# ilovepose/fast-human-pose-estimation.pytorch

Measured on AMD Instinct MI355X. Metric: images/sec FPD train step (4-stack HG student, 8-stack teacher) 256x256, higher is better.
Workload: dtype bf16; 1 GPU; configs[1]: hourglass student S=4 F=128 + teacher S=8 F=256, 256x256, batch 32/GPU, fused FPD step incl. Adam, teacher forward one batch ahead on a 2nd stream; global_batch=32, parallelism=dp1, backend=mfma, launch=one native plan call per phase, kernels launched eagerly on 3 streams, ranks=1, finite=True

## Files before the change

### fast-human-pose-estimation.pytorch_amd/csrc/api.hip

```cpp
#include <cstdarg>
#include <cstdio>
#include <cstdlib>
#include <cstring>
#include <string>
#include <vector>

#include "conv_dispatch.h"

int g_fpd_backend = FPD_BACKEND_MFMA;
static thread_local char g_err[512] = "";

static FILE* g_launch_log_file = nullptr;
static bool launch_log_open() {
    const char* path = getenv("FPD_LAUNCH_LOG");
    if (path == nullptr || path[0] == 0) return false;
    g_launch_log_file = fopen(path, "w");
    if (g_launch_log_file == nullptr) fprintf(stderr, "[fpd_amd] FPD_LAUNCH_LOG: cannot open %s\n", path);
    return g_launch_log_file != nullptr;
}
bool g_fpd_launch_log = launch_log_open();
static thread_local char g_op_tag[256] = "-";
void fpd_log_launch(const char* kernel, const dim3& grid, const dim3& block) {
    if (g_launch_log_file == nullptr) return;
    fprintf(g_launch_log_file, "%s\t%u\t%u\t%s\n", kernel, grid.x * grid.y * grid.z, block.x * block.y * block.z, g_op_tag);
    fflush(g_launch_log_file);
}

int fpd_fail(int code, const char* fmt, ...) {
    va_list ap;
    va_start(ap, fmt);
    vsnprintf(g_err, sizeof(g_err), fmt, ap);
    va_end(ap);
    return code;
}

static int check_launch() {
    hipError_t e = hipGetLastError();
    if (e != hipSuccess) return fpd_fail(-100 - (int)e, "kernel launch failed: %s", hipGetErrorString(e));
    return 0;
}

static int validate_conv_dims(int N, int H, int W, int C, int K, int R, int S, int stride, int pad, int P, int Q) {
    FPD_REQUIRE(N > 0 && H > 0 && W > 0 && C > 0 && K > 0 && R > 0 && S > 0 && stride > 0 && pad >= 0,
                "conv: non-positive dimension");
    FPD_REQUIRE(P == (H + 2 * pad - R) / stride + 1 && Q == (W + 2 * pad - S) / stride + 1,
                "conv: output %dx%d inconsistent with input %dx%d k=%dx%d stride=%d pad=%d", P, Q, H, W, R, S, stride, pad);
    FPD_REQUIRE((int64_t)N * H * W * C < (1ll << 31) && (int64_t)N * P * Q * K < (1ll << 31), "conv: tensor too large for 32-bit indexing");
    return 0;
}

extern "C" {

const char* fpd_last_error(void) { return g_err; }
int fpd_abi_version(void) { return FPD_ABI_VERSION; }
int64_t fpd_stats_words(int32_t channels) { return FPD_STATS_WORDS(channels); }
int fpd_set_backend(int32_t backend) {
    const int prev = g_fpd_backend;
    if (backend == FPD_BACKEND_MFMA || backend == FPD_BACKEND_NAIVE || backend == FPD_BACKEND_MFMA_GENERIC) g_fpd_backend = backend;
    return prev;
}

static int g_wgrad_tile_only = 0;

int fpd_set_option(const char* name, int32_t value) {
    FPD_REQUIRE(name, "set_option: null name");
    if (!strcmp(name, "conv_pp")) return fpd_conv_pp_option(0, value);
    if (!strcmp(name, "conv_pp_blocks")) return fpd_conv_pp_option(1, value);
    if (!strcmp(name, "conv_c1")) return fpd_conv_c1_option(0, value);
    if (!strcmp(name, "conv_c1_blocks")) return fpd_conv_c1_option(1, value);
    if (!strcmp(name, "conv_c1_launches")) return fpd_conv_c1_option(2, value);
    if (!strcmp(name, "conv_skip")) return fpd_conv_c1_option(3, value);
    if (!strcmp(name, "stem_act")) return fpd_stem_s2d_option(0, value);
    if (!strcmp(name, "ew_merge")) return fpd_ew_merge_option(value < 0 ? 0 : value);
    if (!strcmp(name, "ew_merge_blocks")) return fpd_ew_merge_blocks_option(value);
    if (!strcmp(name, "ew_blocks")) return fpd_ew_blocks_option(value);
    if (!strcmp(name, "conv_c3")) return fpd_conv_c3_option(0, value);
    if (!strcmp(name, "conv_c3_blocks")) return fpd_conv_c3_option(1, value);
    if (!strcmp(name, "conv_c3_launches")) return fpd_conv_c3_option(2, value);
    if (!strcmp(name, "bneck_blocks")) return fpd_bneck_blocks_option(value);
    if (!strcmp(name, "bneck_upadd")) return fpd_bneck_upadd_option(value);
    if (!strcmp(name, "head_blocks")) return fpd_head_blocks_option(value);
    if (!strcmp(name, "wgrad_tile_only")) { g_wgrad_tile_only = value; return 0; }
    return fpd_fail(-2, "set_option: unknown option '%s'", name);
}

int fpd_abi_sizeof(const char* n) {
#define SZ(T) if (!strcmp(n, #T)) return (int)sizeof(T)
    SZ(fpd_bn_t); SZ(fpd_conv_t); SZ(fpd_wgrad_t); SZ(fpd_stem_t); SZ(fpd_ew_t); SZ(fpd_loss_t); SZ(fpd_adam_t);
    SZ(fpd_wprep_entry_t); SZ(fpd_bnupd_entry_t); SZ(fpd_memset_t); SZ(fpd_table_t); SZ(fpd_wreduce_entry_t); SZ(fpd_bneck_t); SZ(fpd_conv_pair_t); SZ(fpd_bneck_pair_t); SZ(fpd_ew_pair_t); SZ(fpd_pck_t); SZ(fpd_head_t); SZ(fpd_affsum_t); SZ(fpd_layout_t);
    SZ(fpd_conv_f8_t); SZ(fpd_wquant_entry_t); SZ(fpd_flipmerge_t); SZ(fpd_finalpreds_t); SZ(fpd_targets_t); SZ(fpd_warp_src_t); SZ(fpd_warp_t);
    SZ(fpd_loss_ohkm_t); SZ(fpd_sgd_t); SZ(fpd_ew_merge_t); SZ(fpd_loss_kl_t);
    SZ(fpd_aug_img_t); SZ(fpd_aug_db_t); SZ(fpd_aug_crop_t); SZ(fpd_augment_t); SZ(fpd_warp_aug_t); SZ(fpd_targets_w_t); SZ(fpd_targets_unbiased_t);
    SZ(fpd_oks_nms_t); SZ(fpd_coco_match_t); SZ(fpd_coco_accum_t); SZ(fpd_val_post_t); SZ(fpd_dark_t);
    SZ(fpd_vis_minmax_t); SZ(fpd_vis_max_preds_t); SZ(fpd_vis_joints_grid_t); SZ(fpd_vis_heatmap_grid_t);
#undef SZ
    return -1;
}

static int validate_conv(const fpd_conv_t* a) {
    FPD_REQUIRE(a && a->x && a->w && a->y, "conv: null pointer");
    int rc = validate_conv_dims(a->N, a->H, a->W, a->C, a->K, a->R, a->S, a->stride, a->pad, a->P, a->Q);
    if (rc) return rc;
    FPD_REQUIRE(a->dtype == FPD_F32 || a->dtype == FPD_BF16, "conv: bad dtype %d", a->dtype);
    FPD_REQUIRE(a->bn.mode == FPD_BN_NONE || (a->bn.gamma && a->bn.beta), "conv: BN prologue without gamma/beta");
    FPD_REQUIRE(a->bn.mode != FPD_BN_TRAIN || a->bn.stats, "conv: train-mode BN without statistics");
    FPD_REQUIRE(a->bn.mode != FPD_BN_EVAL || (a->bn.running_mean && a->bn.running_var), "conv: eval-mode BN without running stats");
    FPD_REQUIRE(a->epi == FPD_EPI_PLAIN || (a->epi_x && a->epi_stats && a->epi_bn.mode == FPD_BN_TRAIN && a->epi_bn.stats),
                "conv: BNRELU_BWD epilogue needs epi_x, epi_stats and a train-mode epi_bn");
    FPD_REQUIRE(a->x2 == nullptr || (a->w2 != nullptr && a->C2 > 0), "conv: a second source (x2) needs w2 and C2");
    FPD_REQUIRE(a->x2 == nullptr || a->residual == nullptr, "conv: a second source (x2) and a residual exclude each other");
    return 0;
}

constexpr unsigned ON_MFMA = 1u << FPD_BACKEND_MFMA, ON_GENERIC = ON_MFMA | 1u << FPD_BACKEND_MFMA_GENERIC, ON_ANY = ON_GENERIC | 1u << FPD_BACKEND_NAIVE;
struct ConvBackend {
    const char* name;
    unsigned backends;
    int (*route)(const fpd_conv_t& a, const fpd_conv_t* b, ConvAsk ask, ConvRoute& r);
    int (*launch)(const fpd_conv_t& a, const fpd_conv_t* b, hipStream_t st);
};
static const ConvBackend g_conv_backends[] = {
    {"conv_c1", ON_MFMA, fpd_conv_c1_route, fpd_conv_c1_launch},
    {"conv_c3", ON_MFMA, fpd_conv_c3_route, fpd_conv_c3_launch},
    {"conv_pp", ON_MFMA, fpd_conv_pp_route, fpd_conv_pp_launch},
    {"conv_tile", ON_MFMA, fpd_conv_tile_route, fpd_conv_tile_launch},
    {"conv_mfma", ON_GENERIC, nullptr, [](const fpd_conv_t& a, const fpd_conv_t*, hipStream_t st) { return fpd_conv_mfma_launch(a, st); }},
    {"conv_smallc", ON_GENERIC, nullptr, [](const fpd_conv_t& a, const fpd_conv_t*, hipStream_t st) { return fpd_conv_smallc_launch(a, st); }},
    {"conv_naive", ON_ANY, nullptr, [](const fpd_conv_t& a, const fpd_conv_t*, hipStream_t st) { return fpd_conv_naive_launch(a, st); }},
};
static bool eligible(unsigned backends) { return (backends >> g_fpd_backend & 1u) != 0; }

static const ConvBackend* route_conv(const fpd_conv_t& a, const fpd_conv_t* b, ConvAsk ask, ConvRoute& r) {
    r = ConvRoute{false, 0, 0, false};
    for (const ConvBackend& e : g_conv_backends) {
        if (!eligible(e.backends)) continue;
        if (e.route == nullptr ? b == nullptr : e.route(a, b, ask, r) == 0) return &e;
    }
    return nullptr;
}

static int launch_conv(const fpd_conv_t& a, const fpd_conv_t* b, hipStream_t st) {
    ConvRoute r;
    const ConvBackend* e = route_conv(a, b, fpd_conv_ask(a, b), r);
    if (e == nullptr) {
        const int rc = launch_conv(a, nullptr, st);
        return rc ? rc : launch_conv(*b, nullptr, st);
    }
    FPD_REQUIRE(!(a.wg_partial != nullptr && r.slabs_a == 0) && !(b != nullptr && b->wg_partial != nullptr && r.slabs_b == 0),
                "conv: the launch asks for a fused weight gradient (wg_partial), which its route (%s) does not offer; %s() reports 0 for it",
                e->name, b ? "fpd_conv_pair_fused_wgrad_partials" : "fpd_conv_fused_wgrad_partials");
    FPD_REQUIRE(r.folds || (a.fold_x == nullptr && (b == nullptr || b->fold_x == nullptr)),
                "conv: the launch asks for a folded BN-backward apply (fold_x), which its route (%s) does not offer; %s() reports 0 for it",
                e->name, b ? "fpd_conv_pair_fold_supported" : "fpd_conv_fold_supported");
    FPD_REQUIRE(r.skips || (a.x2 == nullptr && (b == nullptr || b->x2 == nullptr)),
                "conv: the launch carries a second 1x1 source (x2), which its route (%s) does not offer; fpd_conv_skip_supported() reports 0 for it", e->name);
    int rc = e->launch(a, b, st);
    for (++e; rc == 1 && e != std::end(g_conv_backends); ++e)
        if (e->route == nullptr && eligible(e->backends)) rc = e->launch(a, b, st);
    return rc;
}

int fpd_conv_forward(const fpd_conv_t* a, fpd_stream_t stream) {
    int rc = validate_conv(a);
    if (rc) return rc;
    rc = launch_conv(*a, nullptr, (hipStream_t)stream);
    return rc ? rc : check_launch();
}

int fpd_conv_fold_supported(const fpd_conv_t* a) {
    ConvRoute r;
    if (!a || validate_conv(a) != 0) return 0;
    route_conv(*a, nullptr, ConvAsk{true, a->wg_partial != nullptr, a->x2 != nullptr}, r);
    return r.folds ? 1 : 0;
}
int fpd_conv_pair_fold_supported(const fpd_conv_pair_t* p) {
    ConvRoute r;
    if (!p || validate_conv(&p->a) != 0 || validate_conv(&p->b) != 0) return 0;
    if (route_conv(p->a, &p->b, ConvAsk{true, fpd_conv_ask(p->a, &p->b).wg, fpd_conv_ask(p->a, &p->b).skip}, r) != nullptr) return r.folds ? 1 : 0;
    return (fpd_conv_fold_supported(&p->a) && fpd_conv_fold_supported(&p->b)) ? 1 : 0;
}

int fpd_conv_skip_supported(const fpd_conv_t* a) {
    ConvRoute r;
    if (!a || validate_conv(a) != 0) return 0;
    route_conv(*a, nullptr, ConvAsk{a->fold_x != nullptr, a->wg_partial != nullptr, true}, r);
    return r.skips ? 1 : 0;
}

int fpd_conv_fused_wgrad_partials(const fpd_conv_t* a) {
    ConvRoute r;
    if (!a || validate_conv(a) != 0) return 0;
    route_conv(*a, nullptr, ConvAsk{a->fold_x != nullptr, true, a->x2 != nullptr}, r);
    return r.slabs_a;
}
int fpd_conv_pair_fused_wgrad_partials(const fpd_conv_pair_t* p, int32_t* n_a, int32_t* n_b) {
    FPD_REQUIRE(p && n_a && n_b, "conv_pair_fused_wgrad_partials: null pointer");
    *n_a = *n_b = 0;
    if (validate_conv(&p->a) != 0 || validate_conv(&p->b) != 0) return 0;
    ConvRoute r;
    route_conv(p->a, &p->b, ConvAsk{fpd_conv_ask(p->a, &p->b).fold, true, fpd_conv_ask(p->a, &p->b).skip}, r);
    *n_a = r.slabs_a; *n_b = r.slabs_b;
    return 0;
}

int fpd_conv_f8_in_domain(const fpd_conv_t* c) { return (c && fpd_conv_f8_domain(*c)) ? 1 : 0; }

int fpd_conv_forward_f8(const fpd_conv_f8_t* a, fpd_stream_t stream) {
    FPD_REQUIRE(a, "conv_f8: null pointer");
    int rc = validate_conv(&a->c);
    if (rc) return rc;
    FPD_REQUIRE(a->w8 && a->w8_scale, "conv_f8: null fp8 weights / scales");
    FPD_REQUIRE(((uintptr_t)a->w8 & 15) == 0, "conv_f8: w8 must be 16-byte aligned");
    rc = 1;
    if (g_fpd_backend == FPD_BACKEND_MFMA) rc = fpd_conv_tile_f8_launch(a->c, a->w8, a->w8_scale, (hipStream_t)stream);
    if (rc == 1) rc = launch_conv(a->c, nullptr, (hipStream_t)stream);
    return rc ? rc : check_launch();
}

int fpd_weight_quant_f8(const fpd_wquant_entry_t* t, int32_t n, fpd_stream_t stream) {
    FPD_REQUIRE(n == 0 || t != nullptr, "weight_quant_f8: null table");
    int rc = fpd_weight_quant_f8_launch(t, n, (hipStream_t)stream);
    return rc ? rc : check_launch();
}

int fpd_conv_forward_pair(const fpd_conv_pair_t* p, fpd_stream_t stream) {
    FPD_REQUIRE(p, "conv_pair: null pointer");
// ... 513 lines not shown
    return rc ? rc : check_launch();
}

int fpd_weight_prep(const fpd_wprep_entry_t* t, int32_t n, int64_t max_elems, int32_t dtype, fpd_stream_t stream) {
    int rc = fpd_weight_prep_launch(t, n, max_elems, dtype, (hipStream_t)stream);
    return rc ? rc : check_launch();
}
int fpd_bn_update_running(const fpd_bnupd_entry_t* t, int32_t n, fpd_stream_t stream) {
    int rc = fpd_bn_update_running_launch(t, n, (hipStream_t)stream);
    return rc ? rc : check_launch();
}
int fpd_cast(const void* src, void* dst, int64_t n, int32_t sd, int32_t dd, fpd_stream_t stream) {
    int rc = fpd_cast_launch(src, dst, n, sd, dd, (hipStream_t)stream);
    return rc ? rc : check_launch();
}
int fpd_nchw_to_nhwc(const float* src, void* dst, int32_t N, int32_t C, int32_t H, int32_t W, int32_t dtype, fpd_stream_t stream) {
    int rc = fpd_nchw_to_nhwc_launch(src, dst, N, C, H, W, dtype, (hipStream_t)stream);
    return rc ? rc : check_launch();
}
int fpd_nhwc_to_nchw(const void* src, float* dst, int32_t N, int32_t C, int32_t H, int32_t W, int32_t dtype, fpd_stream_t stream) {
    int rc = fpd_nhwc_to_nchw_launch(src, dst, N, C, H, W, dtype, (hipStream_t)stream);
    return rc ? rc : check_launch();
}

struct fpd_op {
    int32_t type;
    union {
        fpd_affsum_t affsum; fpd_layout_t layout; fpd_conv_f8_t conv8; fpd_conv_t conv; fpd_conv_pair_t pair; fpd_bneck_t bneck; fpd_bneck_pair_t bpair; fpd_ew_pair_t epair; fpd_pck_t pck; fpd_head_t head; fpd_wgrad_t wgrad; fpd_stem_t stem; fpd_ew_t ew; fpd_loss_t loss; fpd_loss_ohkm_t lossk; fpd_loss_kl_t losskl; fpd_adam_t adam; fpd_sgd_t sgd; fpd_ew_merge_t ewm;
        fpd_memset_t mset; fpd_table_t table;
    } u;
};
struct fpd_sched {
    int32_t lane = 0;
    bool record = false;
    hipEvent_t done = nullptr;
    std::vector<int32_t> waits;
};
struct fpd_plan {
    std::vector<fpd_op> ops;
    std::vector<fpd_sched> sched;
    std::vector<hipGraphExec_t> graphs;
    std::vector<hipGraph_t> graph_defs;
    hipStream_t lanes[FPD_MAX_LANES] = {};
    hipEvent_t lane_done[FPD_MAX_LANES] = {};
    hipEvent_t fork = nullptr;
};

fpd_plan* fpd_plan_create(void) { return new fpd_plan(); }
void fpd_plan_destroy(fpd_plan* p) {
    if (!p) return;
    for (auto g : p->graphs) (void)hipGraphExecDestroy(g);
    for (auto g : p->graph_defs) (void)hipGraphDestroy(g);
    for (auto& s : p->sched) if (s.done) (void)hipEventDestroy(s.done);
    for (int l = 0; l < FPD_MAX_LANES; ++l) {
        if (p->lanes[l]) (void)hipStreamDestroy(p->lanes[l]);
        if (p->lane_done[l]) (void)hipEventDestroy(p->lane_done[l]);
    }
    if (p->fork) (void)hipEventDestroy(p->fork);
    delete p;
}
int fpd_plan_size(const fpd_plan* p) { return p ? (int)p->ops.size() : -1; }

int fpd_plan_add(fpd_plan* p, int32_t op, const void* args, int64_t bytes) {
    FPD_REQUIRE(p && args, "plan_add: null");
    fpd_op o;
    memset(&o, 0, sizeof(o));
    o.type = op;
    size_t want = 0;
    switch (op) {
        case FPD_OP_CONV: want = sizeof(fpd_conv_t); break;
        case FPD_OP_CONV_F8: want = sizeof(fpd_conv_f8_t); break;
        case FPD_OP_WGRAD: want = sizeof(fpd_wgrad_t); break;
        case FPD_OP_CONV_PAIR: want = sizeof(fpd_conv_pair_t); break;
        case FPD_OP_BNECK_PAIR: want = sizeof(fpd_bneck_pair_t); break;
        case FPD_OP_EW_PAIR: want = sizeof(fpd_ew_pair_t); break;
        case FPD_OP_PCK: want = sizeof(fpd_pck_t); break;
        case FPD_OP_HEAD: case FPD_OP_HEAD_FOLD: want = sizeof(fpd_head_t); break;
        case FPD_OP_BNECK: case FPD_OP_BNECK_FOLD: want = sizeof(fpd_bneck_t); break;
        case FPD_OP_STEM_FWD: case FPD_OP_STEM_WGRAD: want = sizeof(fpd_stem_t); break;
        case FPD_OP_EW: want = sizeof(fpd_ew_t); break;
        case FPD_OP_EW_MERGE: want = sizeof(fpd_ew_merge_t); break;
        case FPD_OP_LOSS: want = sizeof(fpd_loss_t); break;
        case FPD_OP_LOSS_OHKM: want = sizeof(fpd_loss_ohkm_t); break;
        case FPD_OP_LOSS_KL: want = sizeof(fpd_loss_kl_t); break;
        case FPD_OP_ADAM: want = sizeof(fpd_adam_t); break;
        case FPD_OP_SGD: want = sizeof(fpd_sgd_t); break;
        case FPD_OP_MEMSET: case FPD_OP_NOP: want = sizeof(fpd_memset_t); break;
        case FPD_OP_AFFSUM: want = sizeof(fpd_affsum_t); break;
        case FPD_OP_NCHW2NHWC: want = sizeof(fpd_layout_t); break;
        case FPD_OP_WPREP: case FPD_OP_BNUPD: case FPD_OP_WREDUCE: case FPD_OP_WQUANT: want = sizeof(fpd_table_t); break;
        default: return fpd_fail(-2, "plan_add: unknown op %d", op);
    }
    FPD_REQUIRE((size_t)bytes == want, "plan_add: op %d expects %zu bytes of args, got %lld", op, want, (long long)bytes);
    memcpy(&o.u, args, want);
    p->ops.push_back(o);
    p->sched.emplace_back();
    return (int)p->ops.size() - 1;
}

int fpd_plan_set_schedule(fpd_plan* p, int32_t op, int32_t lane, const int32_t* wait_ops, int32_t n_waits) {
    FPD_REQUIRE(p && op >= 0 && op < (int)p->ops.size(), "plan_set_schedule: bad op index %d", op);
    FPD_REQUIRE(lane >= 0 && lane < FPD_MAX_LANES, "plan_set_schedule: lane %d outside [0,%d)", lane, FPD_MAX_LANES);
    FPD_REQUIRE(n_waits >= 0 && (n_waits == 0 || wait_ops != nullptr), "plan_set_schedule: bad wait list");
    for (int i = 0; i < n_waits; ++i)
        FPD_REQUIRE(wait_ops[i] >= 0 && wait_ops[i] < op, "plan_set_schedule: op %d may only wait for earlier ops (got %d)", op, wait_ops[i]);
    fpd_sched& s = p->sched[op];
    s.lane = lane;
    s.waits.assign(wait_ops, wait_ops + n_waits);
    for (int i = 0; i < n_waits; ++i) p->sched[wait_ops[i]].record = true;
    return 0;
}

int fpd_plan_mark_event(fpd_plan* p, int32_t op) {
    FPD_REQUIRE(p && op >= 0 && op < (int)p->ops.size(), "plan_mark_event: bad op index %d", op);
    p->sched[op].record = true;
    return 0;
}

int fpd_plan_wait_op(fpd_plan* p, int32_t op, fpd_stream_t stream) {
    FPD_REQUIRE(p && op >= 0 && op < (int)p->ops.size(), "plan_wait_op: bad op index %d", op);
    FPD_REQUIRE(p->sched[op].record && p->sched[op].done, "plan_wait_op: op %d has no recorded event (mark it, then run its range)", op);
    FPD_CHECK_HIP(hipStreamWaitEvent((hipStream_t)stream, p->sched[op].done, 0));
    return 0;
}

static void conv_tag(char* p, size_t n, const char* what, const fpd_conv_t& c) {
    snprintf(p, n, "%s N=%d H=%d W=%d C=%d K=%d R=%d s=%d %s%s%s%s%s", what, c.N, c.H, c.W, c.C, c.K, c.R, c.stride,
             c.epi == FPD_EPI_BNRELU_BWD ? "dgrad" : "fwd", c.bn.mode == FPD_BN_EVAL ? " evalbn" : "", c.wg_partial ? " +wgrad" : "", c.fold_x ? " +fold" : "",
             c.x2 ? " +skip" : "");
}
static void set_op_tag(int idx, const fpd_op& o) {
    char t[200] = "";
    static const char* ew_names[] = {"bnrelu_fwd", "bnrelu_bwd_r", "bn_bwd_apply", "maxpool_fwd", "maxpool_bwd", "upadd_fwd", "sumpool", "add", "relu_mask", "dilate2"};
    auto ewn = [&](int op) { return (op >= 0 && op < 10) ? ew_names[op] : "ew"; };
    switch (o.type) {
        case FPD_OP_CONV: conv_tag(t, sizeof(t), "conv", o.u.conv); break;
        case FPD_OP_CONV_F8: conv_tag(t, sizeof(t), "conv_f8", o.u.conv8.c); break;
        case FPD_OP_CONV_PAIR: {
            char a[90], b[90];
            conv_tag(a, sizeof(a), "conv2", o.u.pair.a);
            snprintf(b, sizeof(b), " | H=%d W=%d", o.u.pair.b.H, o.u.pair.b.W);
            snprintf(t, sizeof(t), "%s%s", a, b);
            break;
        }
        case FPD_OP_WGRAD: snprintf(t, sizeof(t), "wgrad N=%d H=%d W=%d C=%d K=%d R=%d s=%d", o.u.wgrad.N, o.u.wgrad.H, o.u.wgrad.W, o.u.wgrad.C, o.u.wgrad.K, o.u.wgrad.R, o.u.wgrad.stride); break;
        case FPD_OP_BNECK: snprintf(t, sizeof(t), "bneck N=%d H=%d W=%d C=%d P=%d%s", o.u.bneck.N, o.u.bneck.H, o.u.bneck.W, o.u.bneck.C, o.u.bneck.P, o.u.bneck.x2 ? "+upadd" : ""); break;
        case FPD_OP_BNECK_PAIR: snprintf(t, sizeof(t), "bneck2 N=%d H=%d W=%d C=%d P=%d | H=%d W=%d", o.u.bpair.a.N, o.u.bpair.a.H, o.u.bpair.a.W, o.u.bpair.a.C, o.u.bpair.a.P, o.u.bpair.b.H, o.u.bpair.b.W); break;
        case FPD_OP_HEAD: snprintf(t, sizeof(t), "head N=%d H=%d W=%d C=%d J=%d", o.u.head.N, o.u.head.H, o.u.head.W, o.u.head.C, o.u.head.J); break;
        case FPD_OP_EW: snprintf(t, sizeof(t), "ew %s N=%d H=%d W=%d C=%d", ewn(o.u.ew.op), o.u.ew.N, o.u.ew.H, o.u.ew.W, o.u.ew.C); break;
        case FPD_OP_EW_PAIR: snprintf(t, sizeof(t), "ew2 %s N=%d H=%d W=%d C=%d | H=%d W=%d", ewn(o.u.epair.a.op), o.u.epair.a.N, o.u.epair.a.H, o.u.epair.a.W, o.u.epair.a.C, o.u.epair.b.H, o.u.epair.b.W); break;
        case FPD_OP_EW_MERGE: {
            const fpd_ew_merge_t& m = o.u.ewm;
            const bool pb = m.kind == FPD_EWM_MAXPOOL_BWD;
            snprintf(t, sizeof(t), "ewm %s N=%d H=%d W=%d C=%d", pb ? (m.has_full ? "apply2+maxpool_bwd" : "apply+maxpool_bwd") : "apply+sumpool", m.pool.N, m.pool.H, m.pool.W, m.pool.C);
            break;
        }
        case FPD_OP_STEM_FWD: case FPD_OP_STEM_WGRAD: snprintf(t, sizeof(t), "%s N=%d H=%d W=%d K=%d%s", o.type == FPD_OP_STEM_FWD ? "stem_fwd" : "stem_wgrad", o.u.stem.N, o.u.stem.H, o.u.stem.W, o.u.stem.K,
                                                              (o.type == FPD_OP_STEM_FWD && o.u.stem.act.mode != FPD_BN_NONE) ? " +act" : ""); break;
        case FPD_OP_AFFSUM: snprintf(t, sizeof(t), "affsum N=%d H=%d W=%d C=%d terms=%d", o.u.affsum.N, o.u.affsum.H, o.u.affsum.W, o.u.affsum.C, o.u.affsum.nterms); break;
        case FPD_OP_LOSS: snprintf(t, sizeof(t), "loss B=%d J=%d H=%d W=%d S=%d", o.u.loss.B, o.u.loss.J, o.u.loss.H, o.u.loss.W, o.u.loss.S); break;
        case FPD_OP_LOSS_OHKM: snprintf(t, sizeof(t), "loss_ohkm B=%d J=%d H=%d W=%d S=%d k=%d,%d", o.u.lossk.base.B, o.u.lossk.base.J, o.u.lossk.base.H, o.u.lossk.base.W, o.u.lossk.base.S, o.u.lossk.topk_pose, o.u.lossk.topk_kd); break;
        case FPD_OP_LOSS_KL: snprintf(t, sizeof(t), "loss_kl B=%d J=%d H=%d W=%d S=%d kl=%d,%d T=%g,%g", o.u.losskl.base.B, o.u.losskl.base.J, o.u.losskl.base.H, o.u.losskl.base.W, o.u.losskl.base.S, o.u.losskl.kl_pose, o.u.losskl.kl_kd, (double)o.u.losskl.temp_pose, (double)o.u.losskl.temp_kd); break;
        case FPD_OP_ADAM: snprintf(t, sizeof(t), "adam n=%lld", (long long)o.u.adam.n); break;
        case FPD_OP_SGD: snprintf(t, sizeof(t), "sgd n=%lld momentum=%g wd=%g%s", (long long)o.u.sgd.n, (double)o.u.sgd.momentum, (double)o.u.sgd.weight_decay, o.u.sgd.nesterov ? " nesterov" : ""); break;
        case FPD_OP_WREDUCE: snprintf(t, sizeof(t), "wreduce entries=%d", o.u.table.n); break;
        case FPD_OP_WPREP: snprintf(t, sizeof(t), "wprep entries=%d", o.u.table.n); break;
        case FPD_OP_BNUPD: snprintf(t, sizeof(t), "bnupd entries=%d", o.u.table.n); break;
        default: snprintf(t, sizeof(t), "op%d", o.type); break;
    }
    snprintf(g_op_tag, sizeof(g_op_tag), "%d\t%s", idx, t);
}

static int run_op(const fpd_op& o, fpd_stream_t s) {
    switch (o.type) {
        case FPD_OP_CONV: return fpd_conv_forward(&o.u.conv, s);
        case FPD_OP_CONV_F8: return fpd_conv_forward_f8(&o.u.conv8, s);
        case FPD_OP_WQUANT: return fpd_weight_quant_f8((const fpd_wquant_entry_t*)o.u.table.table, o.u.table.n, s);
        case FPD_OP_WGRAD: return fpd_conv_wgrad(&o.u.wgrad, s);
        case FPD_OP_CONV_PAIR: return fpd_conv_forward_pair(&o.u.pair, s);
        case FPD_OP_BNECK_PAIR: return fpd_bottleneck_forward_pair(&o.u.bpair, s);
        case FPD_OP_EW_PAIR: return fpd_elementwise_pair(&o.u.epair, s);
        case FPD_OP_PCK: return fpd_pck(&o.u.pck, s);
        case FPD_OP_HEAD: return fpd_head_forward(&o.u.head, s);
        case FPD_OP_HEAD_FOLD: return fpd_head_fold(&o.u.head, s);
        case FPD_OP_BNECK: return fpd_bottleneck_forward(&o.u.bneck, s);
        case FPD_OP_BNECK_FOLD: return fpd_bottleneck_fold(&o.u.bneck, s);
        case FPD_OP_STEM_FWD: return fpd_stem_forward(&o.u.stem, s);
        case FPD_OP_STEM_WGRAD: return fpd_stem_wgrad(&o.u.stem, s);
        case FPD_OP_EW: return fpd_elementwise(&o.u.ew, s);
        case FPD_OP_EW_MERGE: return fpd_ew_merge(&o.u.ewm, s);
        case FPD_OP_LOSS: return fpd_loss(&o.u.loss, s);
        case FPD_OP_LOSS_OHKM: return fpd_loss_ohkm(&o.u.lossk, s);
        case FPD_OP_LOSS_KL: return fpd_loss_kl(&o.u.losskl, s);
        case FPD_OP_ADAM: return fpd_adam(&o.u.adam, s);
        case FPD_OP_SGD: return fpd_sgd(&o.u.sgd, s);
        case FPD_OP_MEMSET: {
            FPD_CHECK_HIP(hipMemsetAsync(o.u.mset.ptr, 0, (size_t)o.u.mset.bytes, (hipStream_t)s));
            return 0;
        }
        case FPD_OP_NOP: return 0;
        case FPD_OP_AFFSUM: return fpd_affsum(&o.u.affsum, s);
        case FPD_OP_NCHW2NHWC:
            return fpd_nchw_to_nhwc(o.u.layout.src, o.u.layout.dst, o.u.layout.N, o.u.layout.C, o.u.layout.H, o.u.layout.W, o.u.layout.dtype, s);
        case FPD_OP_WPREP:
            return fpd_weight_prep((const fpd_wprep_entry_t*)o.u.table.table, o.u.table.n, o.u.table.max_elems, o.u.table.dtype, s);
        case FPD_OP_BNUPD: return fpd_bn_update_running((const fpd_bnupd_entry_t*)o.u.table.table, o.u.table.n, s);
        case FPD_OP_WREDUCE: return fpd_wgrad_reduce((const fpd_wreduce_entry_t*)o.u.table.table, o.u.table.n, o.u.table.max_elems, s);
    }
    return fpd_fail(-2, "run_op: unknown op %d", o.type);
}

static int lane_priority() { return 0; }

static int side_streams() { return FPD_MAX_LANES; }

int fpd_plan_run(fpd_plan* p, int32_t begin, int32_t end, fpd_stream_t stream) {
    FPD_REQUIRE(p && begin >= 0 && end <= (int)p->ops.size() && begin <= end, "plan_run: bad range [%d,%d)", begin, end);
    hipStream_t main_s = (hipStream_t)stream;
    bool multi = false;
    for (int i = begin; i < end; ++i) multi |= p->sched[i].lane != 0;
    bool used[FPD_MAX_LANES] = {};
    if (multi) {
        if (!p->fork) FPD_CHECK_HIP(hipEventCreateWithFlags(&p->fork, hipEventDisableTiming));
        FPD_CHECK_HIP(hipEventRecord(p->fork, main_s));
    }
    int rc = 0;
    for (int i = begin; i < end && rc == 0; ++i) {
        fpd_sched& sc = p->sched[i];
        hipStream_t st = main_s;
        if (sc.lane != 0) {
            const int l = 1 + (sc.lane - 1) % side_streams();
            if (!p->lanes[l]) {
                FPD_CHECK_HIP(hipStreamCreateWithPriority(&p->lanes[l], hipStreamNonBlocking, lane_priority()));
                FPD_CHECK_HIP(hipEventCreateWithFlags(&p->lane_done[l], hipEventDisableTiming));
            }
            st = p->lanes[l];
            if (!used[l]) {
                FPD_CHECK_HIP(hipStreamWaitEvent(st, p->fork, 0));
                used[l] = true;
            }
        }
        for (int32_t w : sc.waits)
            if (w >= begin && w < end) FPD_CHECK_HIP(hipStreamWaitEvent(st, p->sched[w].done, 0));
        if (g_fpd_launch_log) set_op_tag(i, p->ops[i]);
        rc = run_op(p->ops[i], (fpd_stream_t)st);
        if (rc) {
            char tmp[400];
            snprintf(tmp, sizeof(tmp), "%s", g_err);
            rc = fpd_fail(rc, "plan op %d (type %d): %s", i, p->ops[i].type, tmp);
            break;
        }
        if (sc.record) {
            if (!sc.done) FPD_CHECK_HIP(hipEventCreateWithFlags(&sc.done, hipEventDisableTiming));
            FPD_CHECK_HIP(hipEventRecord(sc.done, st));
        }
    }
    for (int l = 1; l < FPD_MAX_LANES; ++l)
        if (used[l]) {
            FPD_CHECK_HIP(hipEventRecord(p->lane_done[l], p->lanes[l]));
            FPD_CHECK_HIP(hipStreamWaitEvent(main_s, p->lane_done[l], 0));
        }
    return rc;
}

int fpd_plan_run_op(fpd_plan* p, int32_t op, fpd_stream_t stream) {
    FPD_REQUIRE(p && op >= 0 && op < (int)p->ops.size(), "plan_run_op: bad op index %d", op);
    if (g_fpd_launch_log) set_op_tag(op, p->ops[op]);
    return run_op(p->ops[op], stream);
}

int fpd_plan_capture(fpd_plan* p, int32_t begin, int32_t end, fpd_stream_t stream) {
    FPD_REQUIRE(p, "plan_capture: null");
    FPD_REQUIRE(!g_fpd_launch_log, "plan_capture: FPD_LAUNCH_LOG is set -- the launch log keys a kernel trace 1:1 and cannot follow hipGraph replays; unset one of them");
    hipStream_t st = (hipStream_t)stream;
    FPD_CHECK_HIP(hipStreamBeginCapture(st, hipStreamCaptureModeThreadLocal));
    int rc = fpd_plan_run(p, begin, end, stream);
    hipGraph_t g = nullptr;
    hipError_t e = hipStreamEndCapture(st, &g);
    if (rc) { if (g) (void)hipGraphDestroy(g); return rc; }
    if (e != hipSuccess) return fpd_fail(-100 - (int)e, "hipStreamEndCapture: %s", hipGetErrorString(e));
    hipGraphExec_t ge = nullptr;
    FPD_CHECK_HIP(hipGraphInstantiate(&ge, g, nullptr, nullptr, 0));
    p->graph_defs.push_back(g);
    p->graphs.push_back(ge);
    return (int)p->graphs.size() - 1;
}

int fpd_plan_replay(fpd_plan* p, int32_t gid, fpd_stream_t stream) {
    FPD_REQUIRE(p && gid >= 0 && gid < (int)p->graphs.size(), "plan_replay: bad graph id %d", gid);
    FPD_CHECK_HIP(hipGraphLaunch(p->graphs[gid], (hipStream_t)stream));
    return 0;
}

void* fpd_event_create(void) {
    hipEvent_t e = nullptr;
    if (hipEventCreate(&e) != hipSuccess) return nullptr;
    return (void*)e;
}
int fpd_event_record(void* ev, fpd_stream_t stream) {
    FPD_CHECK_HIP(hipEventRecord((hipEvent_t)ev, (hipStream_t)stream));
    return 0;
}
float fpd_event_elapsed_ms(void* start, void* stop) {
    float ms = -1.f;
    if (hipEventSynchronize((hipEvent_t)stop) != hipSuccess) return -1.f;
    if (hipEventElapsedTime(&ms, (hipEvent_t)start, (hipEvent_t)stop) != hipSuccess) return -1.f;
    return ms;
// ... 5 lines not shown
```

### fast-human-pose-estimation.pytorch_amd/csrc/conv_dispatch.h

```cpp
#pragma once
#include <algorithm>
#include <atomic>
#include <climits>
#include <cstdlib>

#include "common.h"

struct EnvOpt {
    const char* env; int def, lo = INT_MIN, v = -1;
    int get() { if (v < 0) { const char* e = getenv(env); v = e ? atoi(e) : def; } return v < lo ? lo : v; }
    int set(int value) { const int prev = get(); v = value; return prev; }
};

struct GridCap {
    const char* env; int def;
    std::atomic<int> v{0};
    int get() {
        int cap = v.load(std::memory_order_relaxed);
        if (!cap) {
            const char* e = getenv(env);
            cap = std::max(8, e ? atoi(e) : def);
            int unset = 0;
            if (!v.compare_exchange_strong(unset, cap, std::memory_order_relaxed)) cap = unset;
        }
        return cap;
    }
    int set(int value) { get(); return v.exchange(std::max(1, value), std::memory_order_relaxed); }
};

inline int fpd_balanced_blocks(int units, int cap) { return units <= cap ? units : cdiv(units, cdiv(units, cap)); }

inline bool fpd_split_blocks(int ua, int ub, bool pair, int cap, int& na, int& nb) {
    const int total = fpd_balanced_blocks(ua + ub, std::max(1, cap));
    nb = 0;
    if (pair) {
        if (total < 2) return false;
        nb = std::max(1, std::min(total - 1, (int)((long long)total * ub / (ua + ub))));
    }
    na = total - nb;
    return true;
}

struct ConvAsk { bool fold, wg, skip; };
struct ConvRoute { bool folds; int slabs_a, slabs_b; bool skips; };
inline ConvAsk fpd_conv_ask(const fpd_conv_t& a, const fpd_conv_t* b) {
    return ConvAsk{a.fold_x != nullptr || (b != nullptr && b->fold_x != nullptr), a.wg_partial != nullptr || (b != nullptr && b->wg_partial != nullptr),
                   a.x2 != nullptr || (b != nullptr && b->x2 != nullptr)};
}
inline int fpd_conv_check_slabs(const fpd_conv_t& c, int slabs, const char* unit) {
    if (c.wg_partial == nullptr) return 0;
    FPD_REQUIRE(c.wg_stride >= (int64_t)c.C * c.K + c.C, "conv: wg_stride %lld smaller than weight + bias", (long long)c.wg_stride);
    FPD_REQUIRE(c.wg_count == slabs, "conv: the launch writes %d weight-gradient slabs but the caller sized its workspace for %d "
                "(fpd_conv_fused_wgrad_partials: has a %s option changed since?)", slabs, c.wg_count, unit);
    return 0;
}
int fpd_conv_c1_route(const fpd_conv_t& a, const fpd_conv_t* b, ConvAsk ask, ConvRoute& r);
int fpd_conv_c1_launch(const fpd_conv_t& a, const fpd_conv_t* b, hipStream_t st);
int fpd_conv_c3_route(const fpd_conv_t& a, const fpd_conv_t* b, ConvAsk ask, ConvRoute& r);
int fpd_conv_c3_launch(const fpd_conv_t& a, const fpd_conv_t* b, hipStream_t st);
int fpd_conv_pp_route(const fpd_conv_t& a, const fpd_conv_t* b, ConvAsk ask, ConvRoute& r);
int fpd_conv_pp_launch(const fpd_conv_t& a, const fpd_conv_t* b, hipStream_t st);
int fpd_conv_tile_route(const fpd_conv_t& a, const fpd_conv_t* b, ConvAsk ask, ConvRoute& r);
int fpd_conv_tile_launch(const fpd_conv_t& a, const fpd_conv_t* b, hipStream_t st);
int fpd_conv_c1_option(int which, int value);
int fpd_conv_c3_option(int which, int value);
int fpd_conv_pp_option(int which, int value);
int fpd_conv_mfma_launch(const fpd_conv_t& a, hipStream_t st);
int fpd_conv_smallc_launch(const fpd_conv_t& a, hipStream_t st);
int fpd_conv_naive_launch(const fpd_conv_t& a, hipStream_t st);
bool fpd_conv_f8_domain(const fpd_conv_t& a);
int fpd_conv_tile_f8_launch(const fpd_conv_t& a, const void* w8, const float* wscale, hipStream_t st);
int fpd_weight_quant_f8_launch(const fpd_wquant_entry_t* table, int n, hipStream_t st);

int fpd_wgrad_tile_partials(const fpd_wgrad_t& a);
int fpd_wgrad_tile_launch(const fpd_wgrad_t& a, hipStream_t st);
int fpd_wgrad_mfma_partials(const fpd_wgrad_t& a);
int fpd_wgrad_mfma_launch(const fpd_wgrad_t& a, hipStream_t st);
int fpd_wgrad_smallc_partials(const fpd_wgrad_t& a);
int fpd_wgrad_smallc_launch(const fpd_wgrad_t& a, hipStream_t st);
int fpd_wgrad_naive_partials(const fpd_wgrad_t& a);
int fpd_wgrad_naive_launch(const fpd_wgrad_t& a, hipStream_t st);
int fpd_wreduce_launch(const fpd_wreduce_entry_t* table, int n, int64_t max_elems, hipStream_t st);

int fpd_stem_forward_s2d_launch(const fpd_stem_t& a, hipStream_t st);
bool fpd_stem_forward_s2d_takes_act(const fpd_stem_t& a);
int fpd_stem_s2d_option(int which, int value);
int fpd_stem_wgrad_s2d_partials(const fpd_stem_t& a);
int fpd_stem_wgrad_s2d_launch(const fpd_stem_t& a, hipStream_t st);
int fpd_stem_forward_mfma_launch(const fpd_stem_t& a, hipStream_t st);
int fpd_stem_wgrad_mfma_partials(const fpd_stem_t& a);
int fpd_stem_wgrad_mfma_launch(const fpd_stem_t& a, hipStream_t st);
int fpd_stem_forward_launch(const fpd_stem_t& a, hipStream_t st);
int fpd_stem_wgrad_partials(const fpd_stem_t& a);
int fpd_stem_wgrad_launch(const fpd_stem_t& a, hipStream_t st);

int fpd_bneck_fused_launch(const fpd_bneck_t& a, hipStream_t st);
int fpd_bneck_fused_pair_launch(const fpd_bneck_t& a, const fpd_bneck_t& b, hipStream_t st);
int fpd_bneck_fold_launch(const fpd_bneck_t& a, float* out, hipStream_t st);
const char* fpd_bneck_upadd_why_not(const fpd_bneck_t& a);
int fpd_bneck_upadd_option(int value);
int fpd_bneck_blocks_option(int value);
int fpd_head_blocks_option(int value);
int fpd_head_fused_launch(const fpd_head_t& a, hipStream_t st);
int fpd_head_fold_launch(const fpd_head_t& a, float* out, hipStream_t st);
int fpd_pck_launch(const fpd_pck_t& a, hipStream_t st);
int fpd_flip_w_launch(const float* x, float* y, int64_t rows, int W, hipStream_t st);
int fpd_flip_merge_launch(const fpd_flipmerge_t& p, hipStream_t st);
int fpd_final_preds_launch(const fpd_finalpreds_t& p, hipStream_t st);
int fpd_val_post_launch(const fpd_val_post_t& p, hipStream_t st);
int fpd_dark_launch(const fpd_dark_t& p, hipStream_t st);
int fpd_vis_minmax_launch(const fpd_vis_minmax_t& p, hipStream_t st);
int fpd_vis_max_preds_launch(const fpd_vis_max_preds_t& p, hipStream_t st);
int fpd_vis_joints_grid_launch(const fpd_vis_joints_grid_t& p, hipStream_t st);
int fpd_vis_heatmap_grid_launch(const fpd_vis_heatmap_grid_t& p, hipStream_t st);
int64_t fpd_vis_joints_canvas_bytes(const fpd_vis_joints_grid_t& p);
int fpd_render_targets_launch(const fpd_targets_t& a, hipStream_t st);
int fpd_warp_affine_launch(const fpd_warp_t& a, hipStream_t st);
int fpd_render_targets_w_launch(const fpd_targets_w_t& a, hipStream_t st);
int fpd_render_targets_unbiased_launch(const fpd_targets_unbiased_t& a, hipStream_t st);
int fpd_warp_affine_aug_launch(const fpd_warp_aug_t& a, hipStream_t st);
int fpd_augment_params_launch(const fpd_augment_t& a, hipStream_t st);
int fpd_oks_nms_launch(const fpd_oks_nms_t& a, hipStream_t st);
int fpd_coco_match_launch(const fpd_coco_match_t& a, hipStream_t st);
int fpd_coco_accumulate_launch(const fpd_coco_accum_t& a, hipStream_t st);
int fpd_elementwise_launch(const fpd_ew_t& a, hipStream_t st);
int fpd_elementwise_pair_launch(const fpd_ew_t& a, const fpd_ew_t& b, hipStream_t st);
int fpd_affsum_launch(const fpd_affsum_t& a, hipStream_t st);
const char* fpd_ew_merge_why_not(const fpd_ew_merge_t& m);
int fpd_ew_merge_launch(const fpd_ew_merge_t& m, hipStream_t st);
int fpd_ew_merge_option(int value);
int fpd_ew_merge_blocks_option(int value);
int fpd_ew_blocks_option(int value);
int fpd_loss_launch(const fpd_loss_t& a, hipStream_t st);
int fpd_loss_ohkm_launch(const fpd_loss_ohkm_t& a, hipStream_t st);
int64_t fpd_loss_ohkm_scratch_size(const fpd_loss_t& a);
int fpd_loss_kl_launch(const fpd_loss_kl_t& a, hipStream_t st);
int64_t fpd_loss_kl_scratch_size(const fpd_loss_t& a);
int fpd_adam_launch(const fpd_adam_t& a, hipStream_t st);
int fpd_sgd_launch(const fpd_sgd_t& a, hipStream_t st);
int fpd_weight_prep_launch(const fpd_wprep_entry_t* table, int n, int64_t max_elems, int dtype, hipStream_t st);
int fpd_bn_update_running_launch(const fpd_bnupd_entry_t* table, int n, hipStream_t st);
int fpd_cast_launch(const void* src, void* dst, int64_t n, int sd, int dd, hipStream_t st);
int fpd_nchw_to_nhwc_launch(const float* src, void* dst, int N, int C, int H, int W, int dtype, hipStream_t st);
int fpd_nhwc_to_nchw_launch(const void* src, float* dst, int N, int C, int H, int W, int dtype, hipStream_t st);
```

### fast-human-pose-estimation.pytorch_amd/csrc/elementwise.hip

```cpp
#include <algorithm>
#include <cstdlib>

#include "common.h"

namespace {

template <typename T>
__device__ __forceinline__ void ldv(const T* p, float* f) {
    DT<T>::unpack(*reinterpret_cast<const uint4*>(p), f);
}
template <typename T>
__device__ __forceinline__ void stv(T* p, const float* f) {
    *reinterpret_cast<uint4*>(p) = DT<T>::pack(f);
}

template <typename T, bool NA> struct EwPtr { typedef const T* in; typedef T* out; };
template <typename T> struct EwPtr<T, true> { typedef const T* __restrict__ in; typedef T* __restrict__ out; };

template <typename T, int OP, bool NA>
__device__ __forceinline__ void ew_body(const fpd_ew_t& a, const int bx, const int gx) {
    constexpr int VEC = DT<T>::VEC;
    __shared__ float s_t0[FPD_MAXC], s_t1[FPD_MAXC], s_t2[FPD_MAXC], s_t3[FPD_MAXC];
    __shared__ float s_is[FPD_MAXC];
    __shared__ long long s_sum[4 * FPD_MAXC];
// ... 167 lines not shown
        for (int c = tid; c < C; c += 256) stat_flush_lds(dst, s_sum, C, c);
    }
}

template <typename T, int OP, bool NA>
__global__ __launch_bounds__(256) void ew_kernel(const fpd_ew_t a) { ew_body<T, OP, NA>(a, blockIdx.x, gridDim.x); }

static bool ew_no_alias(const fpd_ew_t& a) {
#ifdef FPD_EW_ASSUME_NOALIAS
    return true;
#endif
    return a.y == nullptr || (a.y != a.x && a.y != a.x2 && a.y != a.dy && a.y != a.add);
}

template <typename T, int OP, bool NA>
__global__ __launch_bounds__(256) void ew_pair_kernel(const fpd_ew_t a, const fpd_ew_t b, const int ga) {
    const int gb = (int)gridDim.x - ga;
    if ((int)blockIdx.x < gb) ew_body<T, OP, NA>(b, blockIdx.x, gb);
    else ew_body<T, OP, NA>(a, (int)blockIdx.x - gb, ga);
}

static int ew_stats_blocks() {
    static int v = 0;
    if (!v) {
        const char* e = getenv("FPD_EW_STATS_BLOCKS");
        v = e ? atoi(e) : 512;
        if (v < 1) v = 1;
    }
    return v;
}

int g_ew_blocks = 0;
static int ew_cap(const int grid) { return g_ew_blocks >= 1 ? std::min(grid, g_ew_blocks) : grid; }

template <typename T, int OP>
int ew_rule(const fpd_ew_t& a) {
    constexpr int VEC = DT<T>::VEC;
    const int VP = a.C / VEC, PB = 256 / VP;
    const bool half = (OP == FPD_EW_MAXPOOL_FWD || OP == FPD_EW_MAXPOOL_BWD || OP == FPD_EW_SUMPOOL);
    const int npix = a.N * (half ? a.H / 2 : a.H) * (half ? a.W / 2 : a.W);
    const bool stats = (OP == FPD_EW_BNRELU_FWD || OP == FPD_EW_MAXPOOL_FWD || OP == FPD_EW_UPADD_FWD) ? a.out_stats != nullptr
                                                                                                   : OP == FPD_EW_BNRELU_BWD_R;
    return std::max(1, std::min(cdiv(npix, PB), stats ? ew_stats_blocks() : 2048));
}

template <typename T, int OP>
int ew_grid(const fpd_ew_t& a) { return ew_cap(ew_rule<T, OP>(a)); }

template <typename T, int OP>
int launch_ew(const fpd_ew_t& a, hipStream_t st) {
    const int grid = ew_grid<T, OP>(a);
    if (ew_no_alias(a)) FPD_LAUNCH((ew_kernel<T, OP, true>), dim3(grid), dim3(256), 0, st, a);
    else FPD_LAUNCH((ew_kernel<T, OP, false>), dim3(grid), dim3(256), 0, st, a);
    return 0;
}

template <typename T>
int launch_ew_pair(const fpd_ew_t& a, const fpd_ew_t& b, hipStream_t st) {
    if (a.op != FPD_EW_BN_BWD_APPLY) return 1;
    const int ga = ew_grid<T, FPD_EW_BN_BWD_APPLY>(a), gb = ew_grid<T, FPD_EW_BN_BWD_APPLY>(b);
    if (ew_no_alias(a) && ew_no_alias(b)) FPD_LAUNCH((ew_pair_kernel<T, FPD_EW_BN_BWD_APPLY, true>), dim3(ga + gb), dim3(256), 0, st, a, b, ga);
    else FPD_LAUNCH((ew_pair_kernel<T, FPD_EW_BN_BWD_APPLY, false>), dim3(ga + gb), dim3(256), 0, st, a, b, ga);
    return 0;
}

template <typename T>
__global__ __launch_bounds__(256) void affsum_kernel(const fpd_affsum_t a) {
    constexpr int VEC = DT<T>::VEC;
    __shared__ float s_sc[FPD_AFFSUM_MAX][FPD_MAXC], s_sh[FPD_AFFSUM_MAX][FPD_MAXC];
    const int tid = threadIdx.x;
    const int C = a.C, H = a.H, W = a.W;
    for (int j = 0; j < a.nterms; ++j) {
        if (a.t[j].bn.mode == FPD_BN_NONE) continue;
        const int up = a.t[j].up;
        const double cnt = (double)a.N * (H / up) * (W / up);
        for (int c = tid; c < C; c += 256) {
            float sc, sh, mu, is;
            bn_coef(a.t[j].bn, c, C, cnt, sc, sh, mu, is);
            s_sc[j][c] = sc;
            s_sh[j][c] = sh;
        }
    }
    __syncthreads();
    const int VP = C / VEC, PB = 256 / VP;
    const int cv = (tid % VP) * VEC, pl = tid / VP;
    if (pl >= PB) return;
    const int npix = a.N * H * W;
    T* y = reinterpret_cast<T*>(a.y);
    for (int pix = blockIdx.x * PB + pl; pix < npix; pix += gridDim.x * PB) {
        const int n = pix / (H * W), rem = pix - n * (H * W);
        const int oy = rem / W, ox = rem - oy * W;
        float acc[VEC];
#pragma unroll
        for (int e = 0; e < VEC; ++e) acc[e] = 0.f;
        for (int j = 0; j < a.nterms; ++j) {
            const int up = a.t[j].up;
            const T* x = reinterpret_cast<const T*>(a.t[j].x);
            float v[VEC];
            ldv<T>(x + ((size_t)(n * (H / up) + oy / up) * (W / up) + ox / up) * C + cv, v);
            if (a.t[j].bn.mode != FPD_BN_NONE) {
#pragma unroll
                for (int e = 0; e < VEC; ++e) v[e] = bn_act(v[e], s_sc[j][cv + e], s_sh[j][cv + e], a.t[j].bn.relu);
            }
#pragma unroll
            for (int e = 0; e < VEC; ++e) acc[e] += v[e];
        }
        if (a.relu) {
#pragma unroll
            for (int e = 0; e < VEC; ++e) acc[e] = fmaxf(acc[e], 0.f);
        }
        stv<T>(y + (size_t)pix * C + cv, acc);
    }
}

struct ApplyTab { float t0[FPD_MAXC], t1[FPD_MAXC], t2[FPD_MAXC], mu[FPD_MAXC], is[FPD_MAXC]; };

__device__ __forceinline__ void apply_tab_fill(const fpd_ew_t& a, ApplyTab& t, const int c0, const int stride, const bool grads) {
    const int C = a.C;
    const double cnt = (double)a.N * a.H * a.W;
    for (int c = c0; c < C; c += stride) {
        float sc, sh, mu, is;
        bn_coef(a.bn, c, C, cnt, sc, sh, mu, is);
        t.t0[c] = a.bn.gamma[c] * is;
        const double b1 = stats_sum(a.bstats, C, 0, c), b2 = stats_sum(a.bstats, C, 1, c);
        t.t1[c] = (float)(b1 / cnt);
        t.t2[c] = (float)(b2 / cnt);
        t.mu[c] = mu;
        t.is[c] = is;
        if (grads) {
            if (a.dgamma) a.dgamma[c] = (float)b2;
            if (a.dbeta) a.dbeta[c] = (float)b1;
        }
    }
}

template <typename T>
__device__ __forceinline__ uint4 ldraw(const T* p) { return *reinterpret_cast<const uint4*>(p); }

template <typename T, bool ADD>
__device__ __forceinline__ void apply_vec(const uint4& rg, const uint4& rv, const uint4& rad, const ApplyTab& t, const int cv, float* o) {
    constexpr int VEC = DT<T>::VEC;
    float g[VEC], v[VEC], ad[VEC];
    DT<T>::unpack(rg, g);
    DT<T>::unpack(rv, v);
    if (ADD) DT<T>::unpack(rad, ad);
#pragma unroll
    for (int j = 0; j < VEC; ++j) {
        const int c = cv + j;
        const float xhat = (v[j] - t.mu[c]) * t.is[c];
        o[j] = DT<T>::rnd(t.t0[c] * (g[j] - t.t1[c] - xhat * t.t2[c]) + (ADD ? ad[j] : 0.f));
    }
}

template <typename T, int KIND, bool FULL, bool ADDF, bool ADDH>
__global__ __launch_bounds__(256) void ew_merge_kernel(const fpd_ew_merge_t m) {
    constexpr int VEC = DT<T>::VEC;
    constexpr bool POOLB = KIND == FPD_EWM_MAXPOOL_BWD;
    constexpr bool APF = !POOLB || FULL;
    __shared__ ApplyTab s_f, s_h;
    const int tid = threadIdx.x;
    const int C = m.pool.C, H = m.pool.H, W = m.pool.W, N = m.pool.N;
    if (APF && POOLB) {
        const int w = tid >> 6, c0 = (w >> 1) * 64 + (tid & 63);
        if (w & 1) apply_tab_fill(m.half, s_h, c0, 128, blockIdx.x == 0);
        else apply_tab_fill(m.full, s_f, c0, 128, blockIdx.x == 0);
    } else if (APF) {
        apply_tab_fill(m.full, s_f, tid, 256, blockIdx.x == 0);
    } else {
        apply_tab_fill(m.half, s_h, tid, 256, blockIdx.x == 0);
    }
    __syncthreads();
    const int VP = C / VEC, PB = 256 / VP;
    const int cv = (tid % VP) * VEC, pl = tid / VP;
    if (pl >= PB) return;
    const int OH = H / 2, OW = W / 2, npix = N * OH * OW;
    typedef const T* __restrict__ in_t;
    in_t xf = reinterpret_cast<const T*>(POOLB ? m.pool.x : m.full.x);
    in_t gf = reinterpret_cast<const T*>(m.full.dy);
    in_t af = reinterpret_cast<const T*>(APF ? m.full.add : m.pool.add);
    in_t xh = reinterpret_cast<const T*>(m.half.x);
    in_t gh = reinterpret_cast<const T*>(m.half.dy);
    in_t ah = reinterpret_cast<const T*>(POOLB ? m.half.add : m.pool.add);
    T* __restrict__ const yf = reinterpret_cast<T*>(POOLB ? m.pool.y : m.full.y);
    T* __restrict__ const yh = reinterpret_cast<T*>(m.pool.y);
    for (int pix = blockIdx.x * PB + pl; pix < npix; pix += gridDim.x * PB) {
        const int n = pix / (OH * OW), rem = pix - n * (OH * OW);
        const int oy = rem / OW, ox = rem - oy * OW;
        const size_t ih = (size_t)pix * C + cv;
        const size_t i00 = ((size_t)(n * H + 2 * oy) * W + 2 * ox) * C + cv;
        const size_t i01 = i00 + C, i10 = i00 + (size_t)W * C, i11 = i10 + C;
        const uint4 z = make_uint4(0u, 0u, 0u, 0u);
        uint4 rx0 = z, rx1 = z, rx2 = z, rx3 = z, rg0 = z, rg1 = z, rg2 = z, rg3 = z, ra0 = z, ra1 = z, ra2 = z, ra3 = z, rxh = z, rgh = z, rah = z;
        if (POOLB || APF) { rx0 = ldraw<T>(xf + i00); rx1 = ldraw<T>(xf + i01); rx2 = ldraw<T>(xf + i10); rx3 = ldraw<T>(xf + i11); }
        if (APF) { rg0 = ldraw<T>(gf + i00); rg1 = ldraw<T>(gf + i01); rg2 = ldraw<T>(gf + i10); rg3 = ldraw<T>(gf + i11); }
        if (ADDF) { ra0 = ldraw<T>(af + i00); ra1 = ldraw<T>(af + i01); ra2 = ldraw<T>(af + i10); ra3 = ldraw<T>(af + i11); }
        if (POOLB) { rxh = ldraw<T>(xh + ih); rgh = ldraw<T>(gh + ih); }
        if (ADDH) rah = ldraw<T>(ah + ih);
        float a0[VEC], a1[VEC], a2[VEC], a3[VEC];
        if (APF) {
            apply_vec<T, ADDF>(rg0, rx0, ra0, s_f, cv, a0);
            apply_vec<T, ADDF>(rg1, rx1, ra1, s_f, cv, a1);
            apply_vec<T, ADDF>(rg2, rx2, ra2, s_f, cv, a2);
            apply_vec<T, ADDF>(rg3, rx3, ra3, s_f, cv, a3);
        } else if (ADDF) {
            DT<T>::unpack(ra0, a0); DT<T>::unpack(ra1, a1); DT<T>::unpack(ra2, a2); DT<T>::unpack(ra3, a3);
        } else {
#pragma unroll
            for (int j = 0; j < VEC; ++j) a0[j] = a1[j] = a2[j] = a3[j] = 0.f;
        }
        if (POOLB) {
            float b[VEC], v0[VEC], v1[VEC], v2[VEC], v3[VEC], o0[VEC], o1[VEC], o2[VEC], o3[VEC];
            apply_vec<T, ADDH>(rgh, rxh, rah, s_h, cv, b);
            DT<T>::unpack(rx0, v0); DT<T>::unpack(rx1, v1); DT<T>::unpack(rx2, v2); DT<T>::unpack(rx3, v3);
#pragma unroll
            for (int j = 0; j < VEC; ++j) {
                int arg = 0; float best = v0[j];
                if (v1[j] > best) { best = v1[j]; arg = 1; }
                if (v2[j] > best) { best = v2[j]; arg = 2; }
                if (v3[j] > best) { best = v3[j]; arg = 3; }
                o0[j] = (arg == 0 ? b[j] : 0.f) + a0[j];
                o1[j] = (arg == 1 ? b[j] : 0.f) + a1[j];
                o2[j] = (arg == 2 ? b[j] : 0.f) + a2[j];
                o3[j] = (arg == 3 ? b[j] : 0.f) + a3[j];
            }
            stv<T>(yf + i00, o0); stv<T>(yf + i01, o1); stv<T>(yf + i10, o2); stv<T>(yf + i11, o3);
        } else {
            float ad[VEC], o[VEC];
            if (ADDH) DT<T>::unpack(rah, ad);
#pragma unroll
            for (int j = 0; j < VEC; ++j) o[j] = (a0[j] + a1[j]) + (a2[j] + a3[j]) + (ADDH ? ad[j] : 0.f);
            stv<T>(yf + i00, a0); stv<T>(yf + i01, a1); stv<T>(yf + i10, a2); stv<T>(yf + i11, a3);
            stv<T>(yh + ih, o);
        }
    }
}

int g_ew_merge_blocks = 2048;

template <typename T, int KIND, bool FULL, bool ADDF, bool ADDH>
int launch_ew_merge(const fpd_ew_merge_t& m, hipStream_t st) {
    const int grid = std::min(ew_rule<T, FPD_EW_SUMPOOL>(m.pool), g_ew_merge_blocks);
    FPD_LAUNCH((ew_merge_kernel<T, KIND, FULL, ADDF, ADDH>), dim3(grid), dim3(256), 0, st, m);
    return 0;
}

template <typename T>
int dispatch_ew_merge(const fpd_ew_merge_t& m, hipStream_t st) {
    const bool pb = m.kind == FPD_EWM_MAXPOOL_BWD;
    const bool full = !pb || m.has_full;
    const int v = (pb ? 8 : 0) | (full ? 4 : 0) | ((full ? m.full.add : m.pool.add) ? 2 : 0) | ((pb ? m.half.add : m.pool.add) ? 1 : 0);
    switch (v) {
        case 4: return launch_ew_merge<T, FPD_EWM_SUMPOOL, true, false, false>(m, st);
        case 5: return launch_ew_merge<T, FPD_EWM_SUMPOOL, true, false, true>(m, st);
        case 6: return launch_ew_merge<T, FPD_EWM_SUMPOOL, true, true, false>(m, st);
        case 7: return launch_ew_merge<T, FPD_EWM_SUMPOOL, true, true, true>(m, st);
        case 8: return launch_ew_merge<T, FPD_EWM_MAXPOOL_BWD, false, false, false>(m, st);
        case 9: return launch_ew_merge<T, FPD_EWM_MAXPOOL_BWD, false, false, true>(m, st);
        case 10: return launch_ew_merge<T, FPD_EWM_MAXPOOL_BWD, false, true, false>(m, st);
        case 11: return launch_ew_merge<T, FPD_EWM_MAXPOOL_BWD, false, true, true>(m, st);
        case 12: return launch_ew_merge<T, FPD_EWM_MAXPOOL_BWD, true, false, false>(m, st);
        case 13: return launch_ew_merge<T, FPD_EWM_MAXPOOL_BWD, true, false, true>(m, st);
        case 14: return launch_ew_merge<T, FPD_EWM_MAXPOOL_BWD, true, true, false>(m, st);
        case 15: return launch_ew_merge<T, FPD_EWM_MAXPOOL_BWD, true, true, true>(m, st);
    }
    return fpd_fail(-2, "ew_merge: no variant %d", v);
}

template <typename T>
int dispatch_ew(const fpd_ew_t& a, hipStream_t st) {
    switch (a.op) {
        case FPD_EW_BNRELU_FWD: return launch_ew<T, FPD_EW_BNRELU_FWD>(a, st);
        case FPD_EW_BNRELU_BWD_R: return launch_ew<T, FPD_EW_BNRELU_BWD_R>(a, st);
        case FPD_EW_BN_BWD_APPLY: return launch_ew<T, FPD_EW_BN_BWD_APPLY>(a, st);
        case FPD_EW_MAXPOOL_FWD: return launch_ew<T, FPD_EW_MAXPOOL_FWD>(a, st);
        case FPD_EW_MAXPOOL_BWD: return launch_ew<T, FPD_EW_MAXPOOL_BWD>(a, st);
        case FPD_EW_UPADD_FWD: return launch_ew<T, FPD_EW_UPADD_FWD>(a, st);
        case FPD_EW_SUMPOOL: return launch_ew<T, FPD_EW_SUMPOOL>(a, st);
        case FPD_EW_ADD: return launch_ew<T, FPD_EW_ADD>(a, st);
        case FPD_EW_RELU_MASK: return launch_ew<T, FPD_EW_RELU_MASK>(a, st);
        case FPD_EW_DILATE2: return launch_ew<T, FPD_EW_DILATE2>(a, st);
    }
    return fpd_fail(-2, "elementwise: unknown op %d", a.op);
}

}

static int ew_check(const fpd_ew_t& a) {
    const int vec = (a.dtype == FPD_BF16) ? 8 : 4;
    if (a.C % vec != 0 || a.C > FPD_MAXC || a.C / vec > 128)
        return fpd_fail(-3, "elementwise: C=%d must be a multiple of %d and <= %d", a.C, vec, FPD_MAXC);
    return 0;
}

int fpd_elementwise_pair_launch(const fpd_ew_t& a, const fpd_ew_t& b, hipStream_t st) {
    if (a.op != b.op || a.dtype != b.dtype) return 1;
    int rc = ew_check(a);
    if (rc) return rc;
    rc = ew_check(b);
    if (rc) return rc;
    return a.dtype == FPD_BF16 ? launch_ew_pair<bf16_t>(a, b, st) : launch_ew_pair<float>(a, b, st);
}

int fpd_elementwise_launch(const fpd_ew_t& a, hipStream_t st) {
    const int vec = (a.dtype == FPD_BF16) ? 8 : 4;
    if (a.C % vec != 0 || a.C > FPD_MAXC || a.C / vec > 128)
        return fpd_fail(-3, "elementwise: C=%d must be a multiple of %d and <= %d", a.C, vec, FPD_MAXC);
    const bool pooled = (a.op == FPD_EW_MAXPOOL_FWD || a.op == FPD_EW_MAXPOOL_BWD || a.op == FPD_EW_SUMPOOL ||
                         a.op == FPD_EW_UPADD_FWD || a.op == FPD_EW_DILATE2);
    if (pooled && ((a.H & 1) || (a.W & 1))) return fpd_fail(-3, "elementwise: 2x2 ops need even H,W (got %dx%d)", a.H, a.W);
    return a.dtype == FPD_BF16 ? dispatch_ew<bf16_t>(a, st) : dispatch_ew<float>(a, st);
}

static int ew_merge_default() {
    const char* e = getenv("FPD_EW_MERGE");
    return (e && e[0] == '0' && e[1] == 0) ? 0 : 1;
}
static int g_ew_merge = ew_merge_default();
int fpd_ew_merge_option(int value) {
    const int prev = g_ew_merge;
    if (value >= 0) g_ew_merge = value ? 1 : 0;
    return prev;
}

int fpd_ew_merge_blocks_option(int value) {
    const int prev = g_ew_merge_blocks;
    if (value >= 1) g_ew_merge_blocks = value;
    return prev;
}

int fpd_ew_blocks_option(int value) {
    const int prev = g_ew_blocks;
    if (value >= 0) g_ew_blocks = value;
    return prev;
}

static bool ew_apply_ok(const fpd_ew_t& a, const fpd_ew_t& pool, const int div) {
    return a.op == FPD_EW_BN_BWD_APPLY && a.dtype == pool.dtype && a.N == pool.N && a.H == pool.H / div && a.W == pool.W / div && a.C == pool.C &&
           a.x && a.dy && a.y && a.bstats && a.bn.gamma && a.bn.beta &&
           ((a.bn.mode == FPD_BN_TRAIN && a.bn.stats) || (a.bn.mode == FPD_BN_EVAL && a.bn.running_mean && a.bn.running_var));
}

const char* fpd_ew_merge_why_not(const fpd_ew_merge_t& m) {
    if (fpd_ew_merge_option(-1) == 0) return "switched off (FPD_EW_MERGE=0 / option ew_merge)";
    const fpd_ew_t& p = m.pool;
    if (m.kind != FPD_EWM_MAXPOOL_BWD && m.kind != FPD_EWM_SUMPOOL) return "unknown kind";
    if (p.dtype != FPD_BF16 && p.dtype != FPD_F32) return "bad dtype";
    const int vec = (p.dtype == FPD_BF16) ? 8 : 4;
    if (p.N <= 0 || p.H <= 0 || p.W <= 0 || p.C <= 0 || (p.H & 1) || (p.W & 1)) return "dims must be positive, H and W even";
    if (p.C % vec != 0 || p.C > FPD_MAXC || p.C / vec > 128) return "C must be a multiple of the 16-byte vector and <= FPD_MAXC";
    if ((int64_t)p.N * p.H * p.W * p.C >= ((int64_t)1 << 31)) return "tensor too large for 32-bit pixel indexing";
    const bool pb = m.kind == FPD_EWM_MAXPOOL_BWD;
    if (p.op != (pb ? FPD_EW_MAXPOOL_BWD : FPD_EW_SUMPOOL) || !p.x || !p.y) return "pool member: wrong op or null pointer";
    const void* in[10];
    int n = 0;
    const void* out2 = nullptr;
    if (pb) {
        if (!ew_apply_ok(m.half, p, 2)) return "half-resolution member is not a complete FPD_EW_BN_BWD_APPLY on [N,H/2,W/2,C]";
        if (p.dy != m.half.y) return "the pool backward's dy is not the half-resolution apply's result";
        in[n++] = p.x; in[n++] = m.half.x; in[n++] = m.half.dy; in[n++] = m.half.add;
        if (m.has_full) {
            if (!ew_apply_ok(m.full, p, 1)) return "full-resolution member is not a complete FPD_EW_BN_BWD_APPLY on [N,H,W,C]";
            if (p.add != m.full.y || p.x != m.full.x) return "the pool backward's add / x are not the full-resolution apply's result / input";
            in[n++] = m.full.dy; in[n++] = m.full.add;
        } else {
            in[n++] = p.add;
        }
    } else {
        if (!ew_apply_ok(m.full, p, 1)) return "full-resolution member is not a complete FPD_EW_BN_BWD_APPLY on [N,H,W,C]";
        if (p.x != m.full.y) return "the sum-pool's x is not the apply's result";
        out2 = m.full.y;
        if (out2 == p.y) return "the two outputs are one tensor";
        in[n++] = m.full.x; in[n++] = m.full.dy; in[n++] = m.full.add; in[n++] = p.add;
    }
    for (int i = 0; i < n; ++i)
        if (in[i] != nullptr && (in[i] == p.y || in[i] == out2)) return "an output is one of the inputs";
    for (int i = 0; i < n; ++i)
        if (((uintptr_t)in[i] & 15) != 0) return "pointers must be 16-byte aligned";
    if (((uintptr_t)p.y & 15) != 0 || ((uintptr_t)out2 & 15) != 0) return "pointers must be 16-byte aligned";
    return nullptr;
}

int fpd_ew_merge_launch(const fpd_ew_merge_t& m, hipStream_t st) {
    const char* why = fpd_ew_merge_why_not(m);
    if (why) return fpd_fail(-3, "ew_merge: %s; fpd_ew_merge_supported() reports 0 for it", why);
    return m.pool.dtype == FPD_BF16 ? dispatch_ew_merge<bf16_t>(m, st) : dispatch_ew_merge<float>(m, st);
}

int fpd_affsum_launch(const fpd_affsum_t& a, hipStream_t st) {
    const int vec = (a.dtype == FPD_BF16) ? 8 : 4;
    if (a.C % vec != 0 || a.C > FPD_MAXC || a.C / vec > 128)
        return fpd_fail(-3, "affsum: C=%d must be a multiple of %d and <= %d", a.C, vec, FPD_MAXC);
    const int PB = 256 / (a.C / vec);
    const int grid = ew_cap(std::max(1, std::min(cdiv(a.N * a.H * a.W, PB), 2048)));
    if (a.dtype == FPD_BF16) FPD_LAUNCH((affsum_kernel<bf16_t>), dim3(grid), dim3(256), 0, st, a);
    else FPD_LAUNCH((affsum_kernel<float>), dim3(grid), dim3(256), 0, st, a);
    return 0;
}
```

### fast-human-pose-estimation.pytorch_amd/executor.py

```python
import ctypes as C
import os
from collections import namedtuple

import torch

from . import graph as G
from . import runtime as R
from .schedule import PhaseSchedule

_EW = {'bnrelu_fwd': R.EW_BNRELU_FWD, 'bnrelu_bwd_r': R.EW_BNRELU_BWD_R, 'bn_bwd_apply': R.EW_BN_BWD_APPLY,
       'maxpool_fwd': R.EW_MAXPOOL_FWD, 'maxpool_bwd': R.EW_MAXPOOL_BWD, 'upadd_fwd': R.EW_UPADD_FWD,
       'sumpool': R.EW_SUMPOOL, 'add': R.EW_ADD, 'relu_mask': R.EW_RELU_MASK, 'dilate2': R.EW_DILATE2}
_ARENA_DTYPE = {'param': torch.float32, 'grad': torch.float32, 'rstat': torch.float32, 'nbt': torch.int64,
                'stats': torch.int64, 'losses': torch.float64, 'image': torch.float32, 'target': torch.float32,
                'weight': torch.float32, 'adam_m': torch.float32, 'adam_v': torch.float32, 'fold': torch.float32,
                'w8': torch.uint8, 'w8s': torch.float32, 'ohkm_scratch': torch.float64, 'ohkm_masks': torch.int32,
                'kl_scratch': torch.float64}


def act_torch_dtype(dtype):
    return torch.bfloat16 if dtype == R.BF16 else torch.float32


_STAT_HI, _STAT_LO = float(2 ** 20), float(2 ** 60)
# ... 96 lines not shown
        return True
    if k == 'conv' and h >= 32 and (('no3x3big' in _WHATIF and dims[5] == 3) or ('no1x1big' in _WHATIF and dims[5] == 1)):
        return True
    return ('nobig' in _WHATIF and h >= 64) or ('nomid' in _WHATIF and h == 32) or ('nosmall' in _WHATIF and h <= 16)


class Lowering:

    def __init__(self, arenas, dtype):
        self.A, self.dtype = arenas, dtype
        self.keep = []
        self.use_partials = False
        self.partials, self.partial_elems = {}, 0
        self.fused = set()
        self.reduces = []

    def bn(self, bn):
        s = R.BnT()
        if bn is None:
            s.mode = R.BN_NONE
            return s
        s.mode = R.BN_TRAIN if bn.mode == 'train' else R.BN_EVAL
        s.relu = 1 if bn.relu else 0
        s.eps = G.BN_EPS
        s.stats = self.A.ptr(bn.stats) if bn.mode == 'train' else None
        s.gamma, s.beta = self.A.ptr(bn.gamma), self.A.ptr(bn.beta)
        s.running_mean, s.running_var = self.A.ptr(bn.rmean), self.A.ptr(bn.rvar)
        return s

    def conv(self, op, plain=False):
        if not plain and op.absorbed():
            return _nop()
        s = R.ConvT()
        (s.N, s.H, s.W, s.C, s.K, s.R, s.S, s.stride, s.pad, s.P, s.Q) = op.dims
        s.dtype = self.dtype
        s.epi = R.EPI_BNRELU_BWD if op.epi == 'bnrelu_bwd' else R.EPI_PLAIN
        p = self.A.ptr
        s.x, s.w, s.bias, s.residual, s.y = p(_abuf(op.x)), p(op.w), p(op.bias), p(_abuf(op.residual)), p(_abuf(op.y))
        s.out_stats = p(op.out_stats)
        s.bn = self.bn(op.bn)
        s.epi_x, s.epi_bn, s.epi_stats = p(_abuf(op.epi_x)), self.bn(op.epi_bn), p(op.epi_stats)
        if plain:
            return R.OP_CONV, s
        if op.skip_active:
            self._fill_skip(op, s)
        if op.fused_wgrad is not None and self.use_partials:
            n = R.lib().fpd_conv_fused_wgrad_partials(C.byref(s))
            if n > 0:
                self._fuse_wgrad(op, s, n)
        self._fill_fold(op, s)
        if op.w8 is not None:
            f = R.ConvF8T()
            f.c, f.w8, f.w8_scale = s, p(op.w8), p(op.w8s)
            return R.OP_CONV_F8, f
        return R.OP_CONV, s

    def plan_folds(self, ops):
        if os.environ.get('FPD_FOLD_APPLY', '1') == '0':
            return
        l = R.lib()
        for i, op in enumerate(ops):
            if op is None or op.kind not in ('conv', 'conv2'):
                continue
            cands = [m for m in op.members() if m.fold_apply is not None and not m.fold_apply.folded]
            if not cands or any(m.w8 is not None for m in op.members()):
                continue
            early = False
            for m in cands:
                at = [j for j, _ in _readers_of(ops, m.fold_apply.y, exclude=(m, m.fold_apply, m.fold_wgrad))]
                m.fold_other_readers = bool(at)
                early = early or any(j < i for j in at)
            if early:
                continue
            if op.kind == 'conv2':
                ps = R.ConvPairT()
                ps.a, ps.b = self.conv(op.a, plain=True)[1], self.conv(op.b, plain=True)[1]
                ok = l.fpd_conv_pair_fold_supported(C.byref(ps)) == 1
            else:
                ok = l.fpd_conv_fold_supported(C.byref(self.conv(op, plain=True)[1])) == 1
            if ok:
                for m in cands:
                    m.fold_active = True
                    m.fold_apply.folded = True

    def plan_ew_merge(self, ops):
        if os.environ.get('FPD_EW_MERGE', '1') == '0':
            return
        l = R.lib()
        iv = lambda b: (b.arena, b.off, b.off + b.numel)
        hit = lambda p, q: p[0] == q[0] and p[1] < q[2] and q[1] < p[2]
        is_apply = lambda m: m.kind == 'ew' and m.op == 'bn_bwd_apply' and not m.folded and not m.ewm_absorbed
        lane0 = [i for i, op in enumerate(ops) if op is not None and (op.lane or 0) == 0]
        for k in range(1, len(lane0)):
            i, j = lane0[k - 1], lane0[k]
            prev, op = ops[i], ops[j]
            if op.kind != 'ew' or op.op not in ('maxpool_bwd', 'sumpool') or op.ewm_kind is not None:
                continue
            full = half = None
            if op.op == 'maxpool_bwd':
                cands = [m for m in prev.members() if is_apply(m)] if prev.kind in ('ew', 'ew2') else []
                if len(cands) != len(prev.members()):
                    continue
                half = next((m for m in cands if _abuf(m.y) is _abuf(op.dy)), None)
                full = next((m for m in cands if m is not half), None)
                n, h, w, c = op.dims
                if half is None or tuple(half.dims) != (n, h // 2, w // 2, c):
                    continue
                if full is not None and not (_abuf(op.add) is _abuf(full.y) and _abuf(op.x) is _abuf(full.x) and tuple(full.dims) == tuple(op.dims)):
                    continue
                if any(any(_readers_of(ops, m.y, exclude=(op,))) for m in cands):
                    continue
            else:
                if prev.kind != 'ew' or not is_apply(prev) or _abuf(prev.y) is not _abuf(op.x) or tuple(prev.dims) != tuple(op.dims):
                    continue
                full = prev
                if any(i < at < j for at, _ in _readers_of(ops, full.y)):
                    continue
            group = [m for m in (full, half) if m is not None]
            if not self._ew_merge_intervals_ok(op, full, half, ops[i + 1:j], iv, hit):
                continue
            op.ewm_kind, op.ewm_full, op.ewm_half = op.op, full, half
            if l.fpd_ew_merge_supported(C.byref(self.ew_merge(op)[1])) == 1:
                for m in group:
                    m.ewm_absorbed = True
            else:
                op.ewm_kind = op.ewm_full = op.ewm_half = None

    @staticmethod
    def _ew_merge_intervals_ok(op, full, half, between, iv, hit):
        group = [m for m in (full, half) if m is not None]
        pool_bwd = op.op == 'maxpool_bwd'
        moved_rd, moved_wr = [], []
        for m in group:
            r, w = m.accesses()
            moved_rd += r + [m.bstats]
            moved_wr += [b for b in w if b is not m.bstats and not (pool_bwd and b is _abuf(m.y))]
        ins = moved_rd + [_abuf(t) for t in ((op.x, op.add if full is None else None) if pool_bwd else (op.add,)) if t is not None]
        outs = moved_wr + [_abuf(op.y)]
        if any(hit(iv(o), iv(b)) for o in outs for b in ins):
            return False
        if any(hit(iv(a), iv(b)) for x, a in enumerate(outs) for b in outs[x + 1:]):
            return False
        for top in between:
            if top is None:
                continue
            acc = top.accesses()
            if acc is None:
                return False
            r, w = acc
            if any(hit(iv(a), iv(b)) for a in w for b in moved_rd + moved_wr) or any(hit(iv(a), iv(b)) for a in r for b in moved_wr):
                return False
        return True

    def ew_merge(self, op):
        s = R.EwMergeT()
        s.kind = R.EWM_MAXPOOL_BWD if op.ewm_kind == 'maxpool_bwd' else R.EWM_SUMPOOL
        if op.ewm_full is not None:
            s.has_full, s.full = 1, self.ew(op.ewm_full, plain=True)[1]
        if op.ewm_half is not None:
            s.half = self.ew(op.ewm_half, plain=True)[1]
        s.pool = self.ew(op, plain=True)[1]
        return R.OP_EW_MERGE, s

    def _fill_skip(self, op, s):
        sc, p = op.skip_conv, self.A.ptr
        assert _abuf(sc.y) is _abuf(op.residual) and sc.bn is None, 'skip: the downsample convolution must produce exactly this residual'
        s.x2, s.w2, s.bias2, s.C2 = p(_abuf(sc.x)), p(sc.w), p(sc.bias), sc.dims[3]
        s.residual = None

    def plan_skips(self, ops, readers=None):
        if os.environ.get('FPD_FUSE_SKIP', '1') == '0':
            return
        l = R.lib()
        readers = ops if readers is None else readers
        for op in ops:
            sc = op.skip_conv if op is not None and op.kind == 'conv' else None
            if sc is None or not any(o is sc for o in ops) or (op.lane or 0) != (sc.lane or 0):
                continue
            if op.w8 is not None or sc.w8 is not None or sc.bn is not None:
                continue
            if _abuf(sc.y) is not _abuf(op.residual) or sc.out_stats is not None:
                continue
            if any(_readers_of(readers, sc.y, exclude=(op,))):
                continue
            s = self.conv(op, plain=True)[1]
            self._fill_skip(op, s)
            if l.fpd_conv_skip_supported(C.byref(s)) == 1:
                op.skip_active = True
                sc.skip_fused = True

    def plan_stem_act(self, ops, readers=None):
        if os.environ.get('FPD_STEM_ACT', '1') == '0':
            return
        readers = ops if readers is None else readers
        for op in ops:
            ae = op.act_ew if op is not None and op.kind == 'stem_fwd' else None
            if ae is None or not any(o is ae for o in ops) or (op.lane or 0) != (ae.lane or 0):
                continue
            if ae.op != 'bnrelu_fwd' or ae.bn is None or ae.bn.mode != 'eval' or _abuf(ae.x) is not _abuf(op.y):
                continue
            if op.out_stats is not None or ae.out_stats is not None:
                continue
            if any(_readers_of(readers, op.y, exclude=(ae,))):
                continue
            op.act_active = ae.stem_fused = R.lib().fpd_stem_act_supported(C.byref(self.stem(op, act=True)[1])) == 1

    @staticmethod
    def plan_upadd(ops, readers=None, dtype=R.BF16):
        if os.environ.get('FPD_BNECK_UPADD', '1') == '0':
            return 0
        readers = ops if readers is None else readers
        n = 0
        for op in ops:
            if op is None or op.kind != 'bneck' or op.x2 is not None:
                continue
            ua = getattr(op.x, 'producer', None)
            if ua is None or ua.kind != 'ew' or ua.op != 'upadd_fwd' or ua.out_stats is not None or op.x.stats is not None:
                continue
            if ua.y is not op.x or op.x.persistent or not any(o is ua for o in ops) or (op.lane or 0) != (ua.lane or 0):
                continue
            if [o for _, o in _readers_of(readers, op.x, by_buf=False)] != [op]:
                continue
            s = R.BneckT()
            (s.N, s.H, s.W, s.C, s.P), s.dtype = op.dims, dtype
            if R.lib().fpd_bneck_upadd_supported(C.byref(s)) != 1:
                continue
            op.upadd_op, op.x, op.x2 = ua, ua.x, ua.x2
            ua.upadd_absorbed = True
            n += 1
        return n

    def _fill_fold(self, op, s):
        if not op.fold_active:
            return
        ap, p = op.fold_apply, self.A.ptr
        assert ap.add is None and _abuf(ap.y) is _abuf(op.x), 'fold: the apply must produce exactly this operand'
        s.x = p(_abuf(ap.dy))
        s.fold_x, s.fold_bn, s.fold_stats = p(_abuf(ap.x)), self.bn(ap.bn), p(ap.bstats)
        s.fold_dgamma, s.fold_dbeta = p(ap.dgamma), p(ap.dbeta)
        skip = op.fused_active and not op.fold_other_readers
        s.fold_out = None if skip else p(_abuf(ap.y))

    def _register_slabs(self, wg, s, n, nbias):
        if n > 0:
            numel = wg.dw.numel
            stride = (numel + nbias + 63) // 64 * 64
            self.partials[id(wg)] = Slabs(s, wg.dw, numel, stride, n, self.partial_elems, wg.dbias, nbias)
            self.partial_elems += n * stride

    def _fuse_wgrad(self, op, s, n):
        fw = op.fused_wgrad
        assert fw.dw.numel == s.C * s.K, (fw.dw.numel, s.C, s.K)
        self._register_slabs(fw, s, n, s.C)
        s.wg_bias = 1 if fw.dbias is not None else 0
        s.wg_count = n
        self.fused.add(id(fw))
        op.fused_active = True

    def wquant(self, entries):
        ents = []
        for w, q, sc in entries:
            e = R.WquantEntryT()
            e.w, e.w8, e.scale = self.A.ptr(w), self.A.ptr(q), self.A.ptr(sc)
            e.K, e.RSC = w.shape[0], w.numel // w.shape[0]
            ents.append(e)
        s = R.TableT()
        s.table, s.n, s.dtype, s.max_elems = self._table(ents, R.WquantEntryT), len(ents), self.dtype, 0
        return R.OP_WQUANT, s

    def bneck(self, op):
        s = R.BneckT()
        (s.N, s.H, s.W, s.C, s.P) = op.dims
        s.dtype = self.dtype
        p = self.A.ptr
        s.x, s.y = p(_abuf(op.x)), p(_abuf(op.y))
        s.w1, s.b1, s.w2, s.b2, s.w3, s.b3 = p(op.w1), p(op.b1), p(op.w2), p(op.b2), p(op.w3), p(op.b3)
        s.bn1, s.bn2, s.bn3 = self.bn(op.bn1), self.bn(op.bn2), self.bn(op.bn3)
        s.folded = p(op.folded)
        if op.x2 is not None:
            yb = _abuf(op.y)
            for t in (_abuf(op.x), _abuf(op.x2)):
                assert t.arena != yb.arena or t.off + t.numel <= yb.off or yb.off + yb.numel <= t.off, 'bneck: y overlaps a source of its up-add'
            s.x2 = p(_abuf(op.x2))
        return R.OP_BNECK, s

    def head(self, op):
        s = R.HeadT()
        (s.N, s.H, s.W, s.C, s.J) = op.dims
        s.dtype = self.dtype
        p = self.A.ptr
        s.y0, s.x, s.score, s.next = p(_abuf(op.y0)), p(_abuf(op.x)), p(_abuf(op.score)), p(_abuf(op.next))
        s.w_fc, s.b_fc, s.w_score, s.b_score = p(op.w_fc), p(op.b_fc), p(op.w_score), p(op.b_score)
        s.w_fc2, s.b_fc2, s.w_score2, s.b_score2 = p(op.w_fc2), p(op.b_fc2), p(op.w_score2), p(op.b_score2)
        s.bn = self.bn(op.bn)
        s.folded = p(op.folded)
        return R.OP_HEAD, s

    def wgrad(self, op):
        if id(op) in self.fused:
            return _nop()
        s = R.WgradT()
        (s.N, s.H, s.W, s.C, s.K, s.R, s.S, s.stride, s.pad, s.P, s.Q) = op.dims
        s.dtype = self.dtype
        p = self.A.ptr
        s.x, s.dy, s.dw, s.dbias = p(_abuf(op.x)), p(_abuf(op.dy)), p(op.dw), p(op.dbias)
        s.bn = self.bn(op.bn)
        if self.use_partials:
            self._register_slabs(op, s, R.lib().fpd_wgrad_num_partials(C.byref(s)), s.K)
        return R.OP_WGRAD, s

    def wreduce(self, op):
        if not any(id(w) in self.partials for w in op.wgrads):
            return _nop()
        t = R.TableT()
        self.reduces.append((op, t))
        return R.OP_WREDUCE, t

    def finish_partials(self):
        if not self.partials:
            return
        ws = torch.empty(self.partial_elems, dtype=torch.float32, device=self.A.device)
        self.keep.append(ws)
        for wg, r in self.partials.items():
            if wg in self.fused:
                r.s.wg_partial, r.s.wg_stride = ws.data_ptr() + 4 * r.off, r.stride
            else:
                r.s.partial, r.s.partial_stride = ws.data_ptr() + 4 * r.off, r.stride
        for op, t in self.reduces:
            ents, mx = [], 0
            for w in op.wgrads:
                r = self.partials.get(id(w))
                if r is None:
                    continue
                for at, dst, count in ((r.off, r.dw, r.numel), (r.off + r.numel, r.dbias, r.nbias)):
                    if dst is not None:
                        e = R.WreduceEntryT()
                        e.partial, e.dw, e.n, e.stride, e.count = ws.data_ptr() + 4 * at, self.A.ptr(dst), count, r.stride, r.n
                        ents.append(e)
                mx = max(mx, r.numel)
            t.table, t.n, t.dtype, t.max_elems = self._table(ents, R.WreduceEntryT), len(ents), self.dtype, mx

    def stem(self, op, act=None):
        s = R.StemT()
        (s.N, s.H, s.W, s.K, s.P, s.Q) = op.dims
        s.dtype = self.dtype
        p = self.A.ptr
        s.x = p(op.image)
        if op.kind == 'stem_fwd':
            s.w, s.bias, s.y, s.out_stats = p(op.w), p(op.bias), p(_abuf(op.y)), p(op.out_stats)
            if op.act_active if act is None else act:
                s.act, s.y = self.bn(op.act_ew.bn), p(_abuf(op.act_ew.y))
            return R.OP_STEM_FWD, s
        s.dy, s.dw, s.dbias = p(_abuf(op.dy)), p(op.dw), p(op.dbias)
        if self.use_partials:
            self._register_slabs(op, s, R.lib().fpd_stem_wgrad_num_partials(C.byref(s)), s.K)
        return R.OP_STEM_WGRAD, s

    def ew(self, op, plain=False):
        if op.absorbed(merged=not plain):
            return _nop()
        if not plain and op.ewm_kind is not None:
            return self.ew_merge(op)
        s = R.EwT()
        s.op, s.dtype = _EW[op.op], self.dtype
        (s.N, s.H, s.W, s.C) = op.dims
        p = self.A.ptr
        s.x, s.x2, s.dy, s.add, s.y = p(_abuf(op.x)), p(_abuf(op.x2)), p(_abuf(op.dy)), p(_abuf(op.add)), p(_abuf(op.y))
        s.out_stats, s.bstats, s.dgamma, s.dbeta = p(op.out_stats), p(op.bstats), p(op.dgamma), p(op.dbeta)
        s.bn = self.bn(op.bn)
        return R.OP_EW, s

    def _table(self, entries, cls):
        arr = (cls * len(entries))(*entries)
        raw = torch.frombuffer(bytearray(bytes(arr)), dtype=torch.uint8).to(self.A.device)
        self.keep.append(raw)
        return raw.data_ptr()

    def bnupd(self, op):
        ents = []
        for bn in op.bns:
            e = R.BnupdEntryT()
            e.stats, e.running_mean, e.running_var = self.A.ptr(bn.stats), self.A.ptr(bn.rmean), self.A.ptr(bn.rvar)
            e.num_batches_tracked = self.A.ptr(bn.nbt)
            e.count, e.momentum, e.C = float(bn.count), G.BN_MOMENTUM, bn.C
            ents.append(e)
        s = R.TableT()
        s.table, s.n, s.dtype, s.max_elems = self._table(ents, R.BnupdEntryT), len(ents), self.dtype, 0
        return R.OP_BNUPD, s

    def wprep(self, entries):
        ents, mx = [], 0
        for w, wf, wb in entries:
            e = R.WprepEntryT()
            e.w, e.w_fwd, e.w_bwd = self.A.ptr(w), self.A.ptr(wf), self.A.ptr(wb)
            (e.K, e.R, e.S, e.C) = w.shape
            mx = max(mx, w.numel)
            ents.append(e)
        s = R.TableT()
        s.table, s.n, s.dtype, s.max_elems = self._table(ents, R.WprepEntryT), len(ents), self.dtype, mx
        return R.OP_WPREP, s

    def memset(self, arena_name, off=0, n=None):
        t = self.A.tensor(arena_name)
        n = t.numel() - off if n is None else n
        s = R.MemsetT()
        s.ptr, s.bytes = t.data_ptr() + off * t.element_size(), n * t.element_size()
        return R.OP_MEMSET, s

    def op(self, op):
        if _WHATIF and _whatif_drop(op, getattr(self, 'train', True)):
            return _nop()
        if op.kind == 'conv2':
            s = R.ConvPairT()
            s.a, s.b = self.conv(op.a, plain=True)[1], self.conv(op.b, plain=True)[1]
            if self.use_partials and op.a.fused_wgrad is not None and op.b.fused_wgrad is not None:
                na, nb = C.c_int32(0), C.c_int32(0)
                R.check(R.lib().fpd_conv_pair_fused_wgrad_partials(C.byref(s), C.byref(na), C.byref(nb)), 'fpd_conv_pair_fused_wgrad_partials')
                if na.value > 0 and nb.value > 0:
                    self._fuse_wgrad(op.a, s.a, na.value)
                    self._fuse_wgrad(op.b, s.b, nb.value)
            self._fill_fold(op.a, s.a)
            self._fill_fold(op.b, s.b)
            return R.OP_CONV_PAIR, s
        if op.kind == 'ew2':
            live = [m for m in op.members() if not m.absorbed()]
            if len(live) < 2:
                return self.ew(live[0]) if live else _nop()
            s = R.EwPairT()
            s.a, s.b = self.ew(op.a)[1], self.ew(op.b)[1]
            return R.OP_EW_PAIR, s
        if op.kind == 'bneck2':
            s = R.BneckPairT()
            s.a, s.b = self.bneck(op.a)[1], self.bneck(op.b)[1]
            return R.OP_BNECK_PAIR, s
        if op.kind == 'head_fold':
            return R.OP_HEAD_FOLD, self.head(op.target)[1]
        if op.kind == 'bneck_fold':
            return R.OP_BNECK_FOLD, self.bneck(op.target)[1]
        if op.kind == 'affsum':
            s = R.AffsumT()
            (s.N, s.H, s.W, s.C) = op.dims
            s.dtype, s.relu, s.nterms = self.dtype, 1 if op.relu else 0, len(op.terms)
            assert len(op.terms) <= R.AFFSUM_MAX and op.out_stats is None
            for j, (t, bn, up) in enumerate(op.terms):
                s.t[j].x, s.t[j].bn, s.t[j].up = self.A.ptr(_abuf(t)), self.bn(bn), up
            s.y = self.A.ptr(_abuf(op.y))
            return R.OP_AFFSUM, s
        if op.kind == 'nchw2nhwc':
            s = R.LayoutT()
            (s.N, s.C, s.H, s.W) = op.dims
            s.src, s.dst, s.dtype = self.A.ptr(op.image), self.A.ptr(_abuf(op.y)), self.dtype
            return R.OP_NCHW2NHWC, s
        if op.kind == 'grad_ready':
            return _nop()
        return {'conv': self.conv, 'bneck': self.bneck, 'head': self.head, 'wgrad': self.wgrad, 'wreduce': self.wreduce, 'stem_fwd': self.stem,
                'stem_wgrad': self.stem, 'ew': self.ew, 'bnupd': self.bnupd}[op.kind](op)


class ModelState:

    def __init__(self, table, device, dtype):
        self.table, self.device, self.dtype = table, device, dtype
        self.A = Arenas(device, dtype)
        for name in ('param', 'rstat', 'nbt'):
            self.A.alloc(name, table.sizes[name])
        self.A.alloc('grad', table.sizes['param'])


class GraphInstance:

    def __init__(self, state, cfg, batch, height, width, train, image=None, share_weights_with=None):
        self.state, self.train = state, train
        self._wlp_owner = share_weights_with
        self.dtype = state.dtype
        env = os.environ.get
        if cfg.get('arch') == 'hrnet':
            self.g = G.HRNetGraph(state.table, cfg['extra'], cfg['J'], batch, height, width, train,
                                  wlp_is_master=(self.dtype == R.F32),
                                  wgrad_batch=int(env('FPD_WGRAD_BATCH')) if env('FPD_WGRAD_BATCH') else None,
                                  fp8=bool(cfg.get('fp8', False)))
        else:
            self.g = G.HourglassGraph(state.table, cfg['F'], cfg['S'], cfg['J'], batch, height, width, train,
                                      num_blocks=cfg.get('num_blocks', 1), wlp_is_master=(self.dtype == R.F32),
                                      fuse_bneck=(self.dtype == R.BF16 and not train and env('FPD_FUSE_BNECK', '1') != '0'),
                                      pair_branches=env('FPD_PAIR', '1') != '0', fuse_head=env('FPD_FUSE_HEAD', '1') != '0',
                                      fuse_skip=(self.dtype == R.BF16 and env('FPD_FUSE_SKIP', '1') != '0'),
                                      fuse_stem_act=(self.dtype == R.BF16 and env('FPD_STEM_ACT', '1') != '0'),
                                      wgrad_batch=int(env('FPD_WGRAD_BATCH')) if env('FPD_WGRAD_BATCH') else None)
        self.A = Arenas(state.device, self.dtype, parent=state.A)
        self.low = Lowering(self.A, self.dtype)
        self.low.train = train
        self.plan = R.Plan()
        self.rng = {}
        self.graphs = {}
        self._image_ext = image
        self._finalized = False
        self.mid_ops = []
        self.mid_native = []

    def _schedule(self, name, ir_ops):
        b, e = self.rng[name]
        assert e - b == len(ir_ops), (name, b, e, len(ir_ops))
        if not self.lanes_enabled or not any(o is not None and o.lane for o in ir_ops):
            return
        sch = PhaseSchedule([((o.lane or 0), o.accesses()) if o is not None else (0, None) for o in ir_ops], self.g.n_lanes)
        for k in range(len(ir_ops)):
            if sch.lanes[k] or sch.waits[k]:
                self.plan.set_schedule(b + k, sch.lanes[k], [b + w for w in sch.waits[k]])
        self.schedules[name] = sch

    def finalize(self):
        g = self.g
        ops = g.fwd + self.mid_ops + g.bwd
        self.lanes_enabled = os.environ.get('FPD_LANES', '1') != '0'
        self.schedules = {}
        delay = int(os.environ.get('FPD_REUSE_DELAY', '400')) if self.lanes_enabled else 0
        if not self.train:
            delay = 0
        if not self.train and self.dtype == R.BF16:
            self.low.plan_upadd(g.fwd, readers=ops, dtype=self.dtype)
        act = G.plan_memory(ops, reuse_delay=delay)
        self.act_elems = act
        self.A.alloc('act', act)
        self.A.alloc('stats', g.stats_size)
        if self._wlp_owner is not None:
            o = self._wlp_owner
            assert o.g.wlp_size == g.wlp_size and o.g.fold_size == g.fold_size and not self.train
            self.A.t['wlp'] = o.A.t['wlp']
            self.A.t['fold'] = o.A.t['fold']
        else:
            self.A.alloc('wlp', g.wlp_size)
            self.A.alloc('fold', g.fold_size)
        if self._image_ext is not None:
            self.A.t['image'] = self._image_ext
        else:
            self.A.alloc('image', g.N * 3 * g.H * g.W)
        p = self.plan
        b = len(p)
        p.add(*self.low.memset('stats'))
        entries = []
        for k in self.state.table.conv_keys():
            if k in g.MASTER_ONLY:
                continue
            wf, wb = g.wfwd.get(k), g.wbwd.get(k)
            if wf is not None or wb is not None:
                entries.append((self.state.table[k], wf, wb))
        if entries:
            p.add(*self.low.wprep(entries))
        w8 = getattr(g, 'w8', None)
        if w8:
            self.A.alloc('w8', g.w8_size)
            self.A.alloc('w8s', g.w8s_size)
            p.add(*self.low.wquant([(self.state.table[k], q, sc) for k, (q, sc) in w8.items()]))
        for op in g.fwd:
            for sub in op.members():
                if sub.kind in ('bneck', 'head') and sub.folded is not None:
                    p.add(*self.low.op(G.Op(sub.kind + '_fold', target=sub)))
        self.rng['prep'] = (b, len(p))
        b = len(p)
        self.op_index = {}
        self.low.plan_skips(g.fwd, readers=ops)
        self.low.plan_stem_act(g.fwd, readers=ops)
        for op in g.fwd:
            self.op_index[id(op)] = p.add(*self.low.op(op))
        self.rng['fwd'] = (b, len(p))
        self._schedule('fwd', list(g.fwd))
        b = len(p)
        for fn in self.mid_native:
            fn(p)
        self.rng['mid'] = (b, len(p))
        if self.train:
            b = len(p)
            p.add(*self.low.memset('grad'))
            self.low.use_partials = True
            bwd_ir = [op for op in g.bwd if op.kind != 'seed']
            self.low.plan_folds(bwd_ir)
            if not isinstance(g, G.HRNetGraph):
                self.low.plan_ew_merge(bwd_ir)
            lowered = [self.low.op(op) for op in bwd_ir]
            self.low.finish_partials()
            self.bucket_ops = {}
            for ir, (code, st) in zip(bwd_ir, lowered):
                k = self.op_index[id(ir)] = p.add(code, st)
                if ir.kind == 'grad_ready':
                    self.bucket_ops[ir.bucket] = k
                    p.mark_event(k)
            self.rng['bwd'] = (b, len(p))
            self._schedule('bwd', [None] + bwd_ir)
        self._finalized = True
        return self

    def run(self, name, stream=None):
        gid = self.graphs.get(name)
        if gid is not None:
            self.plan.replay(gid, stream)
            return
        b, e = self.rng[name]
        self.plan.run(b, e, stream)

    def capture(self, names, cap_stream):
        torch.cuda.synchronize()
        with torch.cuda.stream(cap_stream):
            for n in names:
                b, e = self.rng[n]
                self.graphs[n] = self.plan.capture(b, e, C.c_void_p(cap_stream.cuda_stream))
        torch.cuda.synchronize()

    def image(self):
        return self.A.tensor('image').view(self.g.N, 3, self.g.H, self.g.W)

    def calibrate_running_stats(self):
        assert self.train
        torch.cuda.synchronize()
        for bn in self.g.bns:
            st = self.A.stats_read(bn.stats).sum(0)
            mean = st[0] / bn.count
            var = (st[1] / bn.count - mean * mean).clamp_min(0) * (bn.count / max(bn.count - 1, 1))
            self.A.view(bn.rmean).copy_(mean.float())
            self.A.view(bn.rvar).copy_(var.float())

    def output_view(self, i):
        return self.A.view(self.g.outputs[i].buf)

    def out_grad_view(self, i):
        return self.A.view(self.g.out_grads[i].buf)


class FusedFPDStep:

    def __init__(self, student_state, student_cfg, teacher_state, teacher_cfg, batch, height, width, alpha,
                 lr=2.5e-4, betas=(0.9, 0.999), eps=1e-8, world_size=1, adam=None, teacher_chunks=None,
                 use_target_weight=(True, True), ohkm=None, sgd=None, kl=None):
        dev = student_state.device
        if adam is not None and sgd is not None:
            raise R.FpdError('FusedFPDStep: adam= and sgd= are mutually exclusive')
        self.use_w = (bool(use_target_weight[0]), bool(use_target_weight[1]))
        self.dtype = student_state.dtype
        self.alpha, self.world_size = alpha, world_size
        self.B, self.J = batch, student_cfg['J']
        self.ohkm = None
        if ohkm is not None:
            self.ohkm = tuple(self.J if k is None else int(k) for k in ohkm)
            if len(self.ohkm) != 2 or not all(1 <= k <= self.J for k in self.ohkm):
                raise R.FpdError('FusedFPDStep: ohkm=%r: topk must lie in [1, J=%d]' % (ohkm, self.J))
        self.kl = None
        if kl is not None:
            if ohkm is not None:
                raise R.FpdError('FusedFPDStep: kl= and ohkm= are mutually exclusive (no kernel pairs a KL term with hard-keypoint mining)')
            self.kl = tuple(None if t is None else float(t) for t in kl)
            if len(self.kl) != 2 or self.kl == (None, None):
                raise R.FpdError('FusedFPDStep: kl=%r: a pair of temperatures, at least one of them not None' % (kl,))
            if not all(t is None or (0.0 < t < float('inf')) for t in self.kl):
                raise R.FpdError('FusedFPDStep: kl=%r: a temperature must be positive' % (kl,))
        self.teacher = None
        self.teachers = []
        self.tmap = [None, None]
        if teacher_state is not None:
            assert teacher_state.dtype == self.dtype
            if teacher_chunks is None:
                teacher_chunks = 1
            while batch % teacher_chunks:
                teacher_chunks -= 1
            cb = batch // teacher_chunks
            self.teacher = GraphInstance(teacher_state, teacher_cfg, cb, height, width, train=False).finalize()
            self.teachers = [self.teacher] + [
                GraphInstance(teacher_state, teacher_cfg, cb, height, width, train=False,
                              share_weights_with=self.teacher).finalize() for _ in range(1, teacher_chunks)]
            self.teacher.run('prep')
            nt = self.teacher.g.outputs[-1].numel * teacher_chunks
            self.tmap = [torch.zeros(nt, dtype=act_torch_dtype(self.dtype), device=dev) for _ in range(2)]
            self.t_streams = [torch.cuda.Stream(device=dev) for _ in range(teacher_chunks)]
            self.t_stream = self.t_streams[0]
            self.ev_t = [torch.cuda.Event(), torch.cuda.Event()]
            self.ev_chunk = [torch.cuda.Event() for _ in range(teacher_chunks)]
        self._k_t = self._k_s = 0
        self._late_teacher_wait = True
        self.student = GraphInstance(student_state, student_cfg, batch, height, width, train=True)
        g = self.student.g
        self.hh, self.hw = g.outputs[0].shape[1:3]
        A = self.student.A
        A.alloc('target', self.B * self.J * self.hh * self.hw)
        A.alloc('weight', self.B * self.J)
        if self.use_w[0] != self.use_w[1]:
            A.t['weight_kd'] = torch.ones(self.B * self.J, dtype=torch.float32, device=dev)
        if not self.use_w[0]:
            A.tensor('weight').fill_(1.0)
        A.alloc('losses', 4)
        if self.ohkm is not None:
            d = R.LossT()
            d.B, d.J, d.H, d.W, d.S = self.B, self.J, self.hh, self.hw, len(g.outputs)
            nbytes = R.lib().fpd_loss_ohkm_scratch_bytes(d)
            if nbytes < 0:
                R.check(int(nbytes), 'fpd_loss_ohkm_scratch_bytes')
            A.alloc('ohkm_scratch', nbytes // 8)
            A.alloc('ohkm_masks', len(g.outputs) * 2 * self.B)
        if self.kl is not None:
            d = R.LossT()
            d.B, d.J, d.H, d.W, d.S = self.B, self.J, self.hh, self.hw, len(g.outputs)
            nbytes = R.lib().fpd_loss_kl_scratch_bytes(d)
            if nbytes < 0:
                R.check(int(nbytes), 'fpd_loss_kl_scratch_bytes')
            A.alloc('kl_scratch', nbytes // 8)
        self.student.mid_ops = [G.Op('loss', extra_in=list(g.outputs), extra_out=list(g.out_grads))]
        add_loss = self._add_loss_kl if self.kl is not None else self._add_loss if self.ohkm is None else self._add_loss_ohkm
        self.student.mid_native = [lambda plan: add_loss(plan, 0)]
        self.student.finalize()
        b = len(self.student.plan)
        add_loss(self.student.plan, 1)
        self.student.rng['mid1'] = (b, len(self.student.plan))
        n = student_state.table.sizes['param']
        self.n_param = n
        self._dist_work = None
        if sgd is not None:
            self._add_sgd(sgd, student_state, n)
            return
        if adam is not None:
            self.m, self.v, self.lr_dev, self.step_dev = adam.m, adam.v, adam.lr_dev, adam.step_dev
            betas, eps = adam.param_groups[0]['betas'], adam.param_groups[0]['eps']
        else:
            self.m = torch.zeros(n, dtype=torch.float32, device=dev)
            self.v = torch.zeros(n, dtype=torch.float32, device=dev)
            self.lr_dev = torch.full((1,), lr, dtype=torch.float32, device=dev)
            self.step_dev = torch.zeros(1, dtype=torch.int64, device=dev)
        self.betas, self.eps = betas, eps
        a = R.AdamT()
        a.n = n
        pa = student_state.A
        a.param, a.grad = pa.tensor('param').data_ptr(), pa.tensor('grad').data_ptr()
        a.m, a.v = self.m.data_ptr(), self.v.data_ptr()
        a.param_lp = None
        a.lr, a.beta1, a.beta2, a.eps = lr, betas[0], betas[1], eps
# ... 326 lines not shown
```

### fast-human-pose-estimation.pytorch_amd/graph.py

```python
import os
from collections import OrderedDict

BN_EPS = 1e-5
BN_MOMENTUM = 0.1
STATS_REPLICAS = int(os.environ.get('FPD_STATS_REPLICAS', '4'))
WGRAD_LANES = 1
LANE_LEVELS = 0
FOLD_APPLY = os.environ.get('FPD_FOLD_APPLY', '1') != '0'
WREDUCE_MODE = os.environ.get('FPD_WREDUCE_MODE', 'lag')
WGRAD_BATCH = 8


class Buf:
    __slots__ = ('arena', 'off', 'shape', 'name')

    def __init__(self, arena, off, shape, name=''):
        self.arena, self.off, self.shape, self.name = arena, off, tuple(shape), name

    @property
    def numel(self):
        n = 1
        for s in self.shape:
            n *= s
        return n

    def __repr__(self):
        return 'Buf(%s+%s %s %s)' % (self.arena, self.off, self.shape, self.name)


class Act:
    __slots__ = ('shape', 'buf', 'stats', 'producer', 'grad', 'name', 'persistent', 'needs_grad', 'apply_op')

    def __init__(self, shape, name=''):
        self.shape = tuple(shape)
        self.buf = None
        self.stats = None
        self.producer = None
        self.grad = None
        self.name = name
        self.persistent = False
        self.needs_grad = True
        self.apply_op = None

    @property
    def numel(self):
        n, h, w, c = self.shape
        return n * h * w * c


class BN:
    __slots__ = ('name', 'mode', 'relu', 'C', 'gamma', 'beta', 'rmean', 'rvar', 'nbt', 'stats', 'count')

    def __init__(self, name, mode, C, gamma, beta, rmean, rvar, nbt, stats=None, relu=True):
        self.name, self.mode, self.C, self.relu = name, mode, C, relu
        self.gamma, self.beta, self.rmean, self.rvar, self.nbt, self.stats = gamma, beta, rmean, rvar, nbt, stats
        self.count = 0


def f8_conv_domain(dims):
    n, h, w, C, K, R, S, stride, pad, P, Q = dims
    if stride != 1 or R != S or R not in (1, 3) or pad != (R - 1) // 2 or w > 128 or w < 2:
        return False
    if C % 32 or K % 8 or C > 512:
        return False
    bk = 64 if C % 64 == 0 else 32
    return (max(1, 128 // w) + R - 1) * w * (bk // 8) <= 2048


class Op:
    PAIRS = ('conv2', 'ew2', 'bneck2')
    fold_apply = fold_wgrad = fused_wgrad = skip_conv = act_ew = w8 = w8s = folded = ewm_kind = ewm_full = ewm_half = upadd_op = x2 = None
    fold_active = fold_other_readers = fused_active = skip_active = skip_fused = act_active = stem_fused = ewm_absorbed = upadd_absorbed = False

    def __init__(self, kind, **kw):
        self.kind = kind
        self.lane = None
        self.__dict__.update(kw)

    def members(self):
        if self.kind in self.PAIRS:
            return [m for m in (self.a, self.b) if m is not None]
        return [self]

    def absorbed(self, merged=True):
        return bool(self.skip_fused or self.upadd_absorbed or self.stem_fused or (self.kind == 'ew' and self.folded) or (merged and self.ewm_absorbed))

    def accesses(self):
        def b(a):
            return a.buf if isinstance(a, Act) else a

        def bn_bufs(bn):
            if bn is None:
                return []
            return [bn.gamma, bn.beta] + ([bn.stats] if bn.mode == 'train' else [bn.rmean, bn.rvar])
        k = self.kind
        if k in self.PAIRS:
            acc = [m.accesses() for m in self.members()]
            return sum((r for r, _ in acc), []), sum((w for _, w in acc), [])
        if k == 'conv':
            rd = [b(self.x), self.w, self.bias, b(self.residual), b(self.epi_x)] + bn_bufs(self.bn) + bn_bufs(self.epi_bn)
            rd += [self.w8, self.w8s]
            wr = [b(self.y), self.out_stats, self.epi_stats]
            fw, fa, sc = self.fused_wgrad, self.fold_apply, self.skip_conv
            if fw is not None and self.fused_active:
                wr += [fw.dw, fw.dbias]
            if fa is not None and self.fold_active:
                rd += [b(fa.x), b(fa.dy), fa.bstats] + bn_bufs(fa.bn)
                wr += [b(fa.y), fa.dgamma, fa.dbeta]
            if sc is not None and self.skip_active:
                rd += [b(sc.x), sc.w, sc.bias]
        elif k == 'head':
            rd = [b(self.y0), b(self.x), self.w_fc, self.b_fc, self.w_score, self.b_score, self.w_fc2, self.b_fc2,
                  self.w_score2, self.b_score2] + bn_bufs(self.bn)
            wr = [b(self.score), b(self.next)]
        elif k == 'bneck':
            rd = [b(self.x), b(self.x2), self.w1, self.b1, self.w2, self.b2, self.w3, self.b3] + bn_bufs(self.bn1) + \
                bn_bufs(self.bn2) + bn_bufs(self.bn3)
            wr = [b(self.y)]
        elif k == 'wgrad':
            rd = [b(self.x), b(self.dy)] + bn_bufs(self.bn)
            wr = [self.dw, self.dbias]
        elif k == 'affsum':
            rd = [b(t) for t, _, _ in self.terms]
            for _, bn, _ in self.terms:
                rd += bn_bufs(bn)
            wr = [b(self.y), self.out_stats]
        elif k == 'nchw2nhwc':
            rd, wr = [self.image], [b(self.y)]
        elif k == 'wreduce':
            rd, wr = list(self.bufs), list(self.bufs)
        elif k == 'grad_ready':
            rd, wr = [self.region], []
        elif k == 'stem_fwd':
            rd, wr = [self.image, self.w, self.bias], [b(self.y), self.out_stats]
            if self.act_ew is not None and self.act_active:
                rd += bn_bufs(self.act_ew.bn)
                wr += [b(self.act_ew.y)]
        elif k == 'stem_wgrad':
            rd, wr = [self.image, b(self.dy)], [self.dw, self.dbias]
        elif k == 'ew':
            if self.upadd_absorbed:
                return [], []
            rd = [b(self.x), b(self.x2), b(self.dy), b(self.add)] + bn_bufs(self.bn)
            wr = [b(self.y), self.out_stats, self.bstats, self.dgamma, self.dbeta]
            if self.ewm_kind is not None:
                for m in (self.ewm_full, self.ewm_half):
                    if m is not None:
                        rd += [b(m.x), b(m.dy), b(m.add)] + bn_bufs(m.bn)
                        wr += [b(m.y), m.bstats, m.dgamma, m.dbeta]
        else:
            return None
        return [x for x in rd if x is not None], [x for x in wr if x is not None]

    def acts_in(self):
        if self.kind in self.PAIRS:
            return [t for m in self.members() for t in m.acts_in()]
        if self.kind == 'head':
            return [t for t in (self.y0, self.x) if t is not None]
        if self.upadd_absorbed:
            return []
        fa, sc = self.fold_apply, self.skip_conv
        folded = [t for t in (fa.x, fa.dy) if isinstance(t, Act)] if fa is not None else []
        if sc is not None and isinstance(sc.x, Act):
            folded = folded + [sc.x]
        return [getattr(self, f) for f in ('x', 'x2', 'dy', 'add', 'residual', 'epi_x') if
                isinstance(getattr(self, f, None), Act)] + [a for a in getattr(self, 'extra_in', []) if a is not None] + folded

    def acts_out(self):
        if self.kind in self.PAIRS:
            return [t for m in self.members() for t in m.acts_out()]
        if self.kind == 'head':
            return [t for t in (self.score, self.next) if t is not None]
        if self.upadd_absorbed:
            return []
        return [getattr(self, f) for f in ('y',) if isinstance(getattr(self, f, None), Act)] + \
               [a for a in getattr(self, 'extra_out', []) if a is not None] + \
               ([self.act_ew.y] if self.act_ew is not None else [])


class ParamTable:

    def __init__(self, keys, bucket_of=None):
        self.keys = list(keys)
        self.entries = OrderedDict()
        self.logical = dict(self.keys)
        self.sizes = {'param': 0, 'rstat': 0, 'nbt': 0}
        self.bucket = {k: (bucket_of(k) if bucket_of else 0) for k, _ in self.keys}
        placed = {}
        self.buckets = []
        for k, shp in sorted(self.keys, key=lambda ks: self.bucket[ks[0]]):
            if k.endswith('num_batches_tracked'):
                arena = 'nbt'
            elif k.endswith('running_mean') or k.endswith('running_var'):
                arena = 'rstat'
            else:
                arena = 'param'
            n = 1
            for s in shp:
                n *= s
            phys = (shp[0], shp[2], shp[3], shp[1]) if len(shp) == 4 else tuple(shp)
            off = self.sizes[arena]
            placed[k] = Buf(arena, off, phys, k)
            step = 4 if arena != 'nbt' else 2
            self.sizes[arena] = off + (n + step - 1) // step * step
            if arena == 'param':
                b = self.bucket[k]
                while len(self.buckets) <= b:
                    self.buckets.append([off, off])
                self.buckets[b][1] = self.sizes[arena]
        for k, _ in self.keys:
            self.entries[k] = placed[k]
        self.buckets = [tuple(b) for b in self.buckets]

    def __getitem__(self, k):
        return self.entries[k]

    def grad(self, k):
        b = self.entries[k]
        return Buf('grad', b.off, b.shape, 'grad:' + k)

    def conv_keys(self):
        return [k for k, shp in self.keys if len(shp) == 4]

    def trainable_keys(self):
        return [k for k, b in self.entries.items() if b.arena == 'param']

    def grad_bucket(self, b):
        lo, hi = self.buckets[b]
        return Buf('grad', lo, (hi - lo,), 'grad:bucket%d' % b)


def hourglass_bucket_of(num_stacks):
    def f(key):
        p = key.split('.')
        if p[0] in ('hg', 'res', 'fc', 'score', 'fc_', 'score_'):
            return num_stacks - 1 - int(p[1])
        return num_stacks - 1
    return f


def plan_memory(ops, align=64, reuse_delay=0):
    last = {}
    for i, op in enumerate(ops):
        for a in op.acts_in() + op.acts_out():
            last[id(a)] = i
    free = []
    limbo = []
    top = 0

    def alloc(n):
        nonlocal top
        n = (n + align - 1) // align * align
        best = None
        for j, (o, s) in enumerate(free):
            if s >= n and (best is None or s < free[best][1]):
                best = j
        if best is not None:
            o, s = free.pop(best)
            if s > n:
                free.append((o + n, s - n))
            return o, n
        o = top
        top += n
        return o, n

    def release(o, n):
        free.append((o, n))
        free.sort()
        merged = []
        for o2, s2 in free:
            if merged and merged[-1][0] + merged[-1][1] == o2:
                merged[-1] = (merged[-1][0], merged[-1][1] + s2)
            else:
                merged.append((o2, s2))
        free[:] = merged

    sizes = {}
    for i, op in enumerate(ops):
        while limbo and limbo[0][0] + reuse_delay <= i:
            _, o, n = limbo.pop(0)
            release(o, n)
        for a in op.acts_in() + op.acts_out():
            if a.buf is None:
                o, n = alloc(a.numel)
                a.buf = Buf('act', o, a.shape, a.name)
                sizes[id(a)] = n
        seen = set()
        for a in op.acts_in() + op.acts_out():
            if id(a) in seen:
                continue
            seen.add(id(a))
            if last[id(a)] == i and not a.persistent and id(a) in sizes:
                limbo.append((i, a.buf.off, sizes.pop(id(a))))
    return top


class _OpList(list):

    def __init__(self, owner):
        super().__init__()
        self.owner = owner

# ... 660 lines not shown
```

### fast-human-pose-estimation.pytorch_amd/runtime.py

```python
import ctypes as C
import os

_HERE = os.path.dirname(os.path.abspath(__file__))
LIB_PATH = os.environ.get('FPD_AMD_LIB') or os.path.join(_HERE, 'csrc', 'libfpd_amd.so')

F32, BF16 = 0, 1
BN_NONE, BN_TRAIN, BN_EVAL = 0, 1, 2
EPI_PLAIN, EPI_BNRELU_BWD = 0, 1
BACKEND_MFMA, BACKEND_NAIVE, BACKEND_MFMA_GENERIC = 0, 1, 2
(EW_BNRELU_FWD, EW_BNRELU_BWD_R, EW_BN_BWD_APPLY, EW_MAXPOOL_FWD, EW_MAXPOOL_BWD, EW_UPADD_FWD, EW_SUMPOOL,
 EW_ADD, EW_RELU_MASK, EW_DILATE2) = range(10)
(OP_CONV, OP_WGRAD, OP_STEM_FWD, OP_STEM_WGRAD, OP_EW, OP_LOSS, OP_ADAM, OP_MEMSET, OP_WPREP, OP_BNUPD,
 OP_WREDUCE, OP_BNECK, OP_BNECK_FOLD, OP_CONV_PAIR, OP_BNECK_PAIR, OP_EW_PAIR, OP_PCK, OP_HEAD, OP_HEAD_FOLD,
 OP_NOP, OP_AFFSUM, OP_NCHW2NHWC, OP_CONV_F8, OP_WQUANT, OP_LOSS_OHKM, OP_SGD, OP_EW_MERGE, OP_LOSS_KL) = range(28)
EWM_MAXPOOL_BWD, EWM_SUMPOOL = 0, 1
AFFSUM_MAX = 4
MAX_STACKS = 8
MAX_JOINTS = 32
MAXC = 512

_i32, _i64, _f32, _f64, _vp = C.c_int32, C.c_int64, C.c_float, C.c_double, C.c_void_p


class BnT(C.Structure):
    _fields_ = [('mode', _i32), ('relu', _i32), ('eps', _f32), ('_pad', _i32), ('stats', _vp), ('gamma', _vp),
                ('beta', _vp), ('running_mean', _vp), ('running_var', _vp)]


class ConvT(C.Structure):
    _fields_ = [('N', _i32), ('H', _i32), ('W', _i32), ('C', _i32), ('K', _i32), ('R', _i32), ('S', _i32),
                ('stride', _i32), ('pad', _i32), ('P', _i32), ('Q', _i32), ('dtype', _i32), ('epi', _i32),
                ('_pad', _i32), ('x', _vp), ('w', _vp), ('bias', _vp), ('residual', _vp), ('y', _vp),
                ('out_stats', _vp), ('bn', BnT), ('epi_x', _vp), ('epi_bn', BnT), ('epi_stats', _vp),
                ('wg_partial', _vp), ('wg_stride', _i64), ('wg_bias', _i32), ('wg_count', _i32),
                ('fold_x', _vp), ('fold_bn', BnT), ('fold_stats', _vp), ('fold_out', _vp), ('fold_dgamma', _vp), ('fold_dbeta', _vp),
                ('x2', _vp), ('w2', _vp), ('bias2', _vp), ('C2', _i32), ('_pad2', _i32)]


class ConvF8T(C.Structure):
    _fields_ = [('c', ConvT), ('w8', _vp), ('w8_scale', _vp)]


class WquantEntryT(C.Structure):
    _fields_ = [('w', _vp), ('w8', _vp), ('scale', _vp), ('K', _i32), ('RSC', _i32)]


class ConvPairT(C.Structure):
    _fields_ = [('a', ConvT), ('b', ConvT)]


class BneckT(C.Structure):
    _fields_ = [('N', _i32), ('H', _i32), ('W', _i32), ('C', _i32), ('P', _i32), ('dtype', _i32), ('_pad', _i32 * 2),
                ('x', _vp), ('y', _vp), ('w1', _vp), ('b1', _vp), ('w2', _vp), ('b2', _vp), ('w3', _vp), ('b3', _vp),
                ('bn1', BnT), ('bn2', BnT), ('bn3', BnT), ('folded', _vp), ('x2', _vp)]


class BneckPairT(C.Structure):
    _fields_ = [('a', BneckT), ('b', BneckT)]


class WgradT(C.Structure):
    _fields_ = [('N', _i32), ('H', _i32), ('W', _i32), ('C', _i32), ('K', _i32), ('R', _i32), ('S', _i32),
                ('stride', _i32), ('pad', _i32), ('P', _i32), ('Q', _i32), ('dtype', _i32), ('x', _vp), ('dy', _vp),
                ('dw', _vp), ('dbias', _vp), ('bn', BnT), ('partial', _vp), ('partial_stride', _i64)]


class StemT(C.Structure):
    _fields_ = [('N', _i32), ('H', _i32), ('W', _i32), ('K', _i32), ('P', _i32), ('Q', _i32), ('dtype', _i32),
                ('_pad', _i32), ('x', _vp), ('w', _vp), ('bias', _vp), ('y', _vp), ('out_stats', _vp), ('dy', _vp),
                ('dw', _vp), ('dbias', _vp), ('partial', _vp), ('partial_stride', _i64), ('act', BnT)]


class EwT(C.Structure):
    _fields_ = [('op', _i32), ('dtype', _i32), ('N', _i32), ('H', _i32), ('W', _i32), ('C', _i32), ('x', _vp),
                ('x2', _vp), ('dy', _vp), ('add', _vp), ('y', _vp), ('out_stats', _vp), ('bstats', _vp),
                ('dgamma', _vp), ('dbeta', _vp), ('bn', BnT)]


class EwPairT(C.Structure):
    _fields_ = [('a', EwT), ('b', EwT)]


class EwMergeT(C.Structure):
    _fields_ = [('kind', _i32), ('has_full', _i32), ('full', EwT), ('half', EwT), ('pool', EwT)]


class HeadT(C.Structure):
    _fields_ = [('N', _i32), ('H', _i32), ('W', _i32), ('C', _i32), ('J', _i32), ('dtype', _i32), ('_pad', _i32 * 2),
                ('y0', _vp), ('x', _vp), ('score', _vp), ('next', _vp), ('w_fc', _vp), ('b_fc', _vp), ('w_score', _vp),
                ('b_score', _vp), ('w_fc2', _vp), ('b_fc2', _vp), ('w_score2', _vp), ('b_score2', _vp), ('bn', BnT),
                ('folded', _vp)]


class AffTermT(C.Structure):
    _fields_ = [('x', _vp), ('bn', BnT), ('up', _i32), ('_pad', _i32)]


class AffsumT(C.Structure):
    _fields_ = [('N', _i32), ('H', _i32), ('W', _i32), ('C', _i32), ('dtype', _i32), ('relu', _i32), ('nterms', _i32),
                ('_pad', _i32), ('t', AffTermT * 4), ('y', _vp)]


class LayoutT(C.Structure):
    _fields_ = [('src', _vp), ('dst', _vp), ('N', _i32), ('C', _i32), ('H', _i32), ('W', _i32), ('dtype', _i32), ('_pad', _i32)]


class PckT(C.Structure):
    _fields_ = [('B', _i32), ('J', _i32), ('H', _i32), ('W', _i32), ('dtype', _i32), ('log_slots', _i32), ('thr', C.c_float),
                ('_pad', _i32), ('out', _vp), ('target', _vp), ('counts', _vp), ('log', _vp), ('cursor', _vp), ('losses', _vp)]


class FlipMergeT(C.Structure):
    _fields_ = [('N', _i32), ('J', _i32), ('H', _i32), ('W', _i32), ('shift', _i32), ('_pad', _i32), ('a', _vp), ('b', _vp),
                ('y', _vp), ('src', _i32 * 32)]


class FinalPredsT(C.Structure):
    _fields_ = [('N', _i32), ('J', _i32), ('H', _i32), ('W', _i32), ('post_process', _i32), ('_pad', _i32), ('hm', _vp),
                ('trans', _vp), ('coords', _vp), ('preds', _vp), ('maxvals', _vp)]


class ValPostT(C.Structure):
    _fields_ = [('N', _i32), ('J', _i32), ('H', _i32), ('W', _i32), ('dtype', _i32), ('shift', _i32), ('post_process', _i32),
                ('box_f32', _i32), ('row0', _i64), ('rows', _i64), ('a', _vp), ('b', _vp), ('center', _vp), ('scale', _vp),
                ('score', _vp), ('merged', _vp), ('all_preds', _vp), ('all_boxes', _vp), ('src', _i32 * MAX_JOINTS)]


DARK_NCHW, DARK_NHWC = 0, 1
DARK_MIN_KSIZE, DARK_MAX_KSIZE, DARK_MAX_HW = 9, 31, 16384


class DarkT(C.Structure):
    _fields_ = [('N', _i32), ('J', _i32), ('H', _i32), ('W', _i32), ('layout', _i32), ('ksize', _i32), ('box_f32', _i32),
                ('_pad', _i32), ('row0', _i64), ('rows', _i64), ('hm', _vp), ('taps', _vp), ('coords', _vp), ('maxvals', _vp),
                ('refined', _vp), ('trans', _vp), ('preds', _vp), ('center', _vp), ('scale', _vp), ('all_preds', _vp)]


VIS_NCHW, VIS_NHWC = 0, 1


class VisMinmaxT(C.Structure):
    _fields_ = [('n', _i64), ('x', _vp), ('out', _vp)]


class VisMaxPredsT(C.Structure):
    _fields_ = [('N', _i32), ('J', _i32), ('h', _i32), ('w', _i32), ('dtype', _i32), ('layout', _i32), ('hm', _vp),
                ('preds', _vp), ('maxvals', _vp)]


class VisJointsGridT(C.Structure):
    _fields_ = [('N', _i32), ('H', _i32), ('W', _i32), ('J', _i32), ('nrow', _i32), ('padding', _i32), ('joints_f64', _i32),
                ('joints_stride', _i32), ('coord_scale', _f32), ('_pad', _i32), ('canvas_bytes', _i64), ('image', _vp),
                ('minmax', _vp), ('joints', _vp), ('vis', _vp), ('canvas', _vp)]


class VisHeatmapGridT(C.Structure):
    _fields_ = [('N', _i32), ('J', _i32), ('h', _i32), ('w', _i32), ('H', _i32), ('W', _i32), ('dtype', _i32), ('layout', _i32),
                ('normalize', _i32), ('_pad', _i32), ('canvas_bytes', _i64), ('image', _vp), ('minmax', _vp), ('hm', _vp),
                ('preds', _vp), ('table', _vp), ('canvas', _vp)]


class TargetsT(C.Structure):
    _fields_ = [('B', _i32), ('J', _i32), ('H', _i32), ('W', _i32), ('patch', _i32), ('_pad', _i32), ('stride_x', _f64),
                ('stride_y', _f64), ('joints', _vp), ('vis', _vp), ('g', _vp), ('target', _vp), ('weight', _vp)]


class WarpSrcT(C.Structure):
    _fields_ = [('img', _vp), ('h', _i32), ('w', _i32), ('row_bytes', _i64), ('minv', _f64 * 6)]


class WarpT(C.Structure):
    _fields_ = [('B', _i32), ('H', _i32), ('W', _i32), ('_pad', _i32), ('src', _vp), ('mean', _f32 * 3), ('std', _f32 * 3),
                ('out', _vp)]


class AugImgT(C.Structure):
    _fields_ = [('img', _vp), ('h', _i32), ('w', _i32), ('row_bytes', _i64)]


class AugDbT(C.Structure):
    _fields_ = [('N', _i32), ('J', _i32), ('box_f32', _i32), ('_pad', _i32), ('images', _vp), ('joints', _vp), ('vis', _vp),
                ('center', _vp), ('scale', _vp), ('flip_src', _vp), ('upper', _vp), ('aspect_ratio', _f64), ('pixel_std', _f64)]


class AugCropT(C.Structure):
    _fields_ = [('src', _i32), ('flip', _i32), ('minv', _f64 * 6)]


class AugmentT(C.Structure):
    _fields_ = [('db', AugDbT), ('B', _i32), ('is_train', _i32), ('flip', _i32), ('num_joints_half_body', _i32),
                ('idx_stride', _i32), ('draw_stride', _i32), ('out_w', _i32), ('out_h', _i32), ('sf', _f64), ('rf', _f64),
                ('prob_half_body', _f64), ('idx', _vp), ('draws', _vp), ('crop', _vp), ('trans', _vp), ('joints', _vp),
                ('vis', _vp), ('center', _vp), ('scale', _vp), ('rotation', _vp), ('flipped', _vp)]


class WarpAugT(C.Structure):
    _fields_ = [('B', _i32), ('H', _i32), ('W', _i32), ('N', _i32), ('images', _vp), ('crop', _vp), ('mean', _f32 * 3),
                ('std', _f32 * 3), ('out', _vp)]


class TargetsWT(C.Structure):
    _fields_ = [('t', TargetsT), ('joints_weight', _vp)]


class TargetsUnbiasedT(C.Structure):
    _fields_ = [('B', _i32), ('J', _i32), ('H', _i32), ('W', _i32), ('sigma', _i32), ('_pad', _i32), ('stride_x', _f64),
                ('stride_y', _f64), ('joints', _vp), ('vis', _vp), ('joints_weight', _vp), ('target', _vp), ('weight', _vp)]


class OksNmsT(C.Structure):
    _fields_ = [('P_total', _i32), ('n_img', _i32), ('J', _i32), ('soft', _i32), ('rescore', _i32), ('grid', _i32),
                ('in_vis_thre', _f64), ('oks_thre', _f64), ('kpts', _vp), ('area', _vp), ('box_score', _vp), ('offsets', _vp),
                ('sigmas', _vp), ('score', _vp), ('work', _vp), ('keep', _vp), ('n_keep', _vp), ('oks_first', _vp)]


class CocoMatchT(C.Structure):
    _fields_ = [('n_img', _i32), ('J', _i32), ('G_total', _i32), ('D_total', _i32), ('grid', _i32), ('_pad', _i32),
                ('oks_total', _i64), ('area_lo', _f64 * 3), ('area_hi', _f64 * 3), ('oks_thrs', _f64 * 10), ('gt_kpts', _vp),
                ('gt_area', _vp), ('gt_bbox', _vp), ('gt_flags', _vp), ('dt_kpts', _vp), ('gt_offsets', _vp), ('dt_offsets', _vp),
                ('oks_offsets', _vp), ('sigmas', _vp), ('oks', _vp), ('scratch', _vp), ('matched', _vp), ('dt_ignored', _vp),
                ('gt_counted', _vp), ('dt_area', _vp), ('status', _vp)]


class CocoAccumT(C.Structure):
    _fields_ = [('D_total', _i32), ('n_rec', _i32), ('matched', _vp), ('dt_ignored', _vp), ('order', _vp), ('npig', _vp),
                ('rec_thrs', _vp), ('tp', _vp), ('env', _vp), ('precision', _vp), ('recall', _vp), ('status', _vp)]


class LossT(C.Structure):
# ... 265 lines not shown
```

### include/fpd_amd.h

```cpp
#ifndef FPD_AMD_H
#define FPD_AMD_H

#include <stddef.h>
#include <stdint.h>

#ifdef __cplusplus
extern "C" {
#endif

typedef void* fpd_stream_t;

enum { FPD_F32 = 0, FPD_BF16 = 1 };
#ifndef FPD_STATS_REPLICAS
#define FPD_STATS_REPLICAS 4
#endif
typedef int64_t fpd_stat_t;
#define FPD_STATS_WORDS(C) ((int64_t)FPD_STATS_REPLICAS * 4 * (C))
enum { FPD_BN_NONE = 0, FPD_BN_TRAIN = 1, FPD_BN_EVAL = 2 };
enum { FPD_EPI_PLAIN = 0, FPD_EPI_BNRELU_BWD = 1 };
enum { FPD_BACKEND_MFMA = 0, FPD_BACKEND_NAIVE = 1, FPD_BACKEND_MFMA_GENERIC = 2 };

typedef struct {
    int32_t mode;
    int32_t relu;
    float eps;
    int32_t _pad;
    const fpd_stat_t* stats;
    const float* gamma;
    const float* beta;
    const float* running_mean;
    const float* running_var;
} fpd_bn_t;

typedef struct {
    int32_t N, H, W, C;
    int32_t K, R, S;
    int32_t stride, pad;
    int32_t P, Q;
    int32_t dtype;
    int32_t epi;
    int32_t _pad;
    const void* x;
    const void* w;
    const float* bias;
    const void* residual;
    void* y;
    fpd_stat_t* out_stats;
    fpd_bn_t bn;
    const void* epi_x;
    fpd_bn_t epi_bn;
    fpd_stat_t* epi_stats;
    float* wg_partial;
    int64_t wg_stride;
    int32_t wg_bias;
    int32_t wg_count;
    const void* fold_x;
    fpd_bn_t fold_bn;
    const fpd_stat_t* fold_stats;
    void* fold_out;
    float* fold_dgamma;
    float* fold_dbeta;
    const void* x2;
    const void* w2;
    const float* bias2;
    int32_t C2;
    int32_t _pad2;
} fpd_conv_t;

typedef struct {
    int32_t N, H, W, C, P, dtype;
    int32_t _pad[2];
    const void* x;
    void* y;
    const void* w1;
    const float* b1;
    const void* w2;
    const float* b2;
    const void* w3;
    const float* b3;
    fpd_bn_t bn1, bn2, bn3;
    const float* folded;
    const void* x2;
} fpd_bneck_t;

typedef struct {
    int32_t N, H, W, C, J, dtype;
    int32_t _pad[2];
    const void* y0;
    const void* x;
    void* score;
    void* next;
    const void* w_fc;
    const float* b_fc;
    const void* w_score;
    const float* b_score;
    const void* w_fc2;
    const float* b_fc2;
    const void* w_score2;
    const float* b_score2;
    fpd_bn_t bn;
    const float* folded;
} fpd_head_t;
int fpd_head_forward(const fpd_head_t* a, fpd_stream_t stream);
int fpd_head_fold(const fpd_head_t* a, fpd_stream_t stream);

typedef struct { fpd_conv_t a, b; } fpd_conv_pair_t;

typedef struct { fpd_bneck_t a, b; } fpd_bneck_pair_t;

typedef struct {
    int32_t N, H, W, C, K, R, S, stride, pad, P, Q, dtype;
    const void* x;
    const void* dy;
    float* dw;
    float* dbias;
    fpd_bn_t bn;
    float* partial;
    int64_t partial_stride;
} fpd_wgrad_t;

typedef struct {
    int32_t N, H, W, K, P, Q, dtype, _pad;
    const float* x;
    const float* w;
    const float* bias;
    void* y;
    fpd_stat_t* out_stats;
    const void* dy;
    float* dw;
    float* dbias;
    float* partial;
    int64_t partial_stride;
    fpd_bn_t act;
} fpd_stem_t;

enum {
    FPD_EW_BNRELU_FWD = 0, FPD_EW_BNRELU_BWD_R = 1, FPD_EW_BN_BWD_APPLY = 2, FPD_EW_MAXPOOL_FWD = 3,
    FPD_EW_MAXPOOL_BWD = 4, FPD_EW_UPADD_FWD = 5, FPD_EW_SUMPOOL = 6, FPD_EW_ADD = 7, FPD_EW_RELU_MASK = 8,
    FPD_EW_DILATE2 = 9
};
typedef struct {
    int32_t op, dtype;
    int32_t N, H, W, C;
    const void* x;
    const void* x2;
    const void* dy;
    const void* add;
    void* y;
    fpd_stat_t* out_stats;
    fpd_stat_t* bstats;
    float* dgamma;
    float* dbeta;
    fpd_bn_t bn;
} fpd_ew_t;

enum { FPD_EWM_MAXPOOL_BWD = 0, FPD_EWM_SUMPOOL = 1 };
typedef struct {
    int32_t kind;
    int32_t has_full;
    fpd_ew_t full;
    fpd_ew_t half;
    fpd_ew_t pool;
} fpd_ew_merge_t;
int fpd_ew_merge(const fpd_ew_merge_t* a, fpd_stream_t stream);
int fpd_ew_merge_supported(const fpd_ew_merge_t* a);

#define FPD_AFFSUM_MAX 4
typedef struct { const void* x; fpd_bn_t bn; int32_t up; int32_t _pad; } fpd_affterm_t;
typedef struct {
    int32_t N, H, W, C;
    int32_t dtype, relu, nterms, _pad;
    fpd_affterm_t t[FPD_AFFSUM_MAX];
    void* y;
} fpd_affsum_t;
int fpd_affsum(const fpd_affsum_t* a, fpd_stream_t stream);

typedef struct { const float* src; void* dst; int32_t N, C, H, W, dtype, _pad; } fpd_layout_t;

#define FPD_MAX_STACKS 8
typedef struct {
    int32_t B, J, H, W, S, dtype;
    int32_t target_nchw;
    float alpha;
    const void* out[FPD_MAX_STACKS];
    void* dout[FPD_MAX_STACKS];
    const void* teacher;
    const float* target;
    const float* weight;
    double* losses;
    float grad_scale;
    int32_t _pad;
    const float* weight_kd;
} fpd_loss_t;

typedef struct {
    fpd_loss_t base;
    int32_t topk_pose, topk_kd;
    void* scratch;
    int64_t scratch_bytes;
    uint32_t* masks;
} fpd_loss_ohkm_t;

typedef struct {
    fpd_loss_t base;
    int32_t kl_pose, kl_kd;
    float temp_pose, temp_kd;
    void* scratch;
    int64_t scratch_bytes;
} fpd_loss_kl_t;

typedef struct {
    int64_t n;
    float* param; const float* grad; float* m; float* v;
    void* param_lp;
    float lr, beta1, beta2, eps;
    float bias_corr1, bias_corr2;
    float grad_scale;
    int32_t _pad;
    const float* lr_dev;
    int64_t* step_dev;
} fpd_adam_t;

typedef struct {
    int64_t n;
    float* param; const float* grad; float* buf;
    void* param_lp;
    float lr, momentum, weight_decay;
    float grad_scale;
    int32_t nesterov;
    int32_t _pad;
    const float* lr_dev;
    int64_t* step_dev;
} fpd_sgd_t;

typedef struct {
    const float* w;
    void* w_fwd;
    void* w_bwd;
    int32_t K, R, S, C;
} fpd_wprep_entry_t;

typedef struct {
    const fpd_stat_t* stats;
    float* running_mean; float* running_var; int64_t* num_batches_tracked;
    double count; float momentum; int32_t C;
} fpd_bnupd_entry_t;

typedef struct {
    const float* partial; float* dw; int64_t n; int64_t stride; int32_t count; int32_t _pad;
} fpd_wreduce_entry_t;

int fpd_conv_forward(const fpd_conv_t* a, fpd_stream_t stream);
int fpd_conv_forward_pair(const fpd_conv_pair_t* p, fpd_stream_t stream);
int fpd_bottleneck_forward(const fpd_bneck_t* a, fpd_stream_t stream);
int fpd_bottleneck_fold(const fpd_bneck_t* a, fpd_stream_t stream);
int fpd_bottleneck_forward_pair(const fpd_bneck_pair_t* p, fpd_stream_t stream);
int fpd_bneck_upadd_supported(const fpd_bneck_t* a);
int fpd_conv_fused_wgrad_partials(const fpd_conv_t* a);
int fpd_conv_fold_supported(const fpd_conv_t* a);
int fpd_conv_pair_fold_supported(const fpd_conv_pair_t* p);
int fpd_conv_skip_supported(const fpd_conv_t* a);
int fpd_conv_pair_fused_wgrad_partials(const fpd_conv_pair_t* p, int32_t* n_a, int32_t* n_b);
int fpd_conv_wgrad(const fpd_wgrad_t* a, fpd_stream_t stream);
int fpd_wgrad_num_partials(const fpd_wgrad_t* a);
int fpd_wgrad_reduce(const fpd_wreduce_entry_t* table_dev, int32_t n_entries, int64_t max_elems, fpd_stream_t stream);
int fpd_stem_forward(const fpd_stem_t* a, fpd_stream_t stream);
int fpd_stem_act_supported(const fpd_stem_t* a);
int fpd_stem_wgrad(const fpd_stem_t* a, fpd_stream_t stream);
int fpd_stem_wgrad_num_partials(const fpd_stem_t* a);
int fpd_elementwise(const fpd_ew_t* a, fpd_stream_t stream);
typedef struct { fpd_ew_t a, b; } fpd_ew_pair_t;
int fpd_elementwise_pair(const fpd_ew_pair_t* p, fpd_stream_t stream);
int fpd_loss(const fpd_loss_t* a, fpd_stream_t stream);
int fpd_loss_ohkm(const fpd_loss_ohkm_t* a, fpd_stream_t stream);
int64_t fpd_loss_ohkm_scratch_bytes(const fpd_loss_t* a);
int fpd_loss_kl(const fpd_loss_kl_t* a, fpd_stream_t stream);
int64_t fpd_loss_kl_scratch_bytes(const fpd_loss_t* a);
int fpd_adam(const fpd_adam_t* a, fpd_stream_t stream);
int fpd_sgd(const fpd_sgd_t* a, fpd_stream_t stream);
int fpd_weight_prep(const fpd_wprep_entry_t* table_dev, int32_t n_entries, int64_t max_elems, int32_t dtype,
                    fpd_stream_t stream);
int fpd_bn_update_running(const fpd_bnupd_entry_t* table_dev, int32_t n_entries, fpd_stream_t stream);
int fpd_cast(const void* src, void* dst, int64_t n, int32_t src_dtype, int32_t dst_dtype, fpd_stream_t stream);
int fpd_nchw_to_nhwc(const float* src, void* dst, int32_t N, int32_t C, int32_t H, int32_t W, int32_t dtype,
                     fpd_stream_t stream);
int fpd_nhwc_to_nchw(const void* src, float* dst, int32_t N, int32_t C, int32_t H, int32_t W, int32_t dtype,
                     fpd_stream_t stream);

typedef struct {
    int32_t B, J, H, W, dtype, log_slots;
    float thr;
    int32_t _pad;
    const void* out;
    const float* target;
    float* counts;
    double* log;
    long long* cursor;
    const double* losses;
} fpd_pck_t;
int fpd_pck(const fpd_pck_t* a, fpd_stream_t stream);

typedef struct {
    fpd_conv_t c;
    const void* w8;
    const float* w8_scale;
} fpd_conv_f8_t;
int fpd_conv_forward_f8(const fpd_conv_f8_t* a, fpd_stream_t stream);
int fpd_conv_f8_in_domain(const fpd_conv_t* c);

// ... 326 lines not shown
```

Before: 3864 images/s.

## Fold residual adds and BN-backward applies into merged elementwise backward kernels

Adds a planner pass over the backward graph that absorbs a preceding elementwise add into the maxpool-backward merge kernel as a second addend (add2). It also fuses a bn_bwd_apply followed by a bnrelu_bwd_r into a single new kernel that applies the gradient, masks it, and accumulates the BN backward sums. The goal is fewer kernel launches and fewer full-resolution activation round-trips through memory. In exchange the planner needs extra aliasing and interval checks, and the fused kernel carries more shared-memory tables, so occupancy may drop.

Measured after the change: 3869 images/s (median of 3 runs). About the same (+0.1%).

```diff
diff --git a/fast-human-pose-estimation.pytorch_amd/csrc/api.hip b/fast-human-pose-estimation.pytorch_amd/csrc/api.hip
--- a/fast-human-pose-estimation.pytorch_amd/csrc/api.hip
+++ b/fast-human-pose-estimation.pytorch_amd/csrc/api.hip
@@ -72,6 +72,7 @@
     if (!strcmp(name, "conv_skip")) return fpd_conv_c1_option(3, value);
     if (!strcmp(name, "stem_act")) return fpd_stem_s2d_option(0, value);
     if (!strcmp(name, "ew_merge")) return fpd_ew_merge_option(value < 0 ? 0 : value);
+    if (!strcmp(name, "fold_rest")) return fpd_fold_rest_option(value < 0 ? 0 : value);
     if (!strcmp(name, "ew_merge_blocks")) return fpd_ew_merge_blocks_option(value);
     if (!strcmp(name, "ew_blocks")) return fpd_ew_blocks_option(value);
     if (!strcmp(name, "conv_c3")) return fpd_conv_c3_option(0, value);
@@ -891,7 +892,8 @@
         case FPD_OP_EW_MERGE: {
             const fpd_ew_merge_t& m = o.u.ewm;
             const bool pb = m.kind == FPD_EWM_MAXPOOL_BWD;
-            snprintf(t, sizeof(t), "ewm %s N=%d H=%d W=%d C=%d", pb ? (m.has_full ? "apply2+maxpool_bwd" : "apply+maxpool_bwd") : "apply+sumpool", m.pool.N, m.pool.H, m.pool.W, m.pool.C);
+            snprintf(t, sizeof(t), "ewm %s%s N=%d H=%d W=%d C=%d", m.kind == FPD_EWM_BNRELU_BWD_R ? "apply+bnrelu_bwd_r" : pb ? (m.has_full ? "apply2+maxpool_bwd" : "apply+maxpool_bwd") : "apply+sumpool",
+                     m.full.add2 ? "+add2" : "", m.pool.N, m.pool.H, m.pool.W, m.pool.C);
             break;
         }
         case FPD_OP_STEM_FWD: case FPD_OP_STEM_WGRAD: snprintf(t, sizeof(t), "%s N=%d H=%d W=%d K=%d%s", o.type == FPD_OP_STEM_FWD ? "stem_fwd" : "stem_wgrad", o.u.stem.N, o.u.stem.H, o.u.stem.W, o.u.stem.K,
diff --git a/fast-human-pose-estimation.pytorch_amd/csrc/conv_dispatch.h b/fast-human-pose-estimation.pytorch_amd/csrc/conv_dispatch.h
--- a/fast-human-pose-estimation.pytorch_amd/csrc/conv_dispatch.h
+++ b/fast-human-pose-estimation.pytorch_amd/csrc/conv_dispatch.h
@@ -129,6 +129,7 @@
 const char* fpd_ew_merge_why_not(const fpd_ew_merge_t& m);
 int fpd_ew_merge_launch(const fpd_ew_merge_t& m, hipStream_t st);
 int fpd_ew_merge_option(int value);
+int fpd_fold_rest_option(int value);
 int fpd_ew_merge_blocks_option(int value);
 int fpd_ew_blocks_option(int value);
 int fpd_loss_launch(const fpd_loss_t& a, hipStream_t st);
diff --git a/fast-human-pose-estimation.pytorch_amd/csrc/elementwise.hip b/fast-human-pose-estimation.pytorch_amd/csrc/elementwise.hip
--- a/fast-human-pose-estimation.pytorch_amd/csrc/elementwise.hip
+++ b/fast-human-pose-estimation.pytorch_amd/csrc/elementwise.hip
@@ -343,7 +343,18 @@
     }
 }
 
-template <typename T, int KIND, bool FULL, bool ADDF, bool ADDH>
+template <typename T>
+__device__ __forceinline__ uint4 add_raw(const uint4& ra, const uint4& rb) {
+    constexpr int VEC = DT<T>::VEC;
+    float v[VEC], u[VEC], o[VEC];
+    DT<T>::unpack(ra, v);
+    DT<T>::unpack(rb, u);
+#pragma unroll
+    for (int j = 0; j < VEC; ++j) o[j] = v[j] + u[j];
+    return DT<T>::pack(o);
+}
+
+template <typename T, int KIND, bool FULL, bool ADDF, bool ADDH, bool ADD2 = false>
 __global__ __launch_bounds__(256) void ew_merge_kernel(const fpd_ew_merge_t m) {
     constexpr int VEC = DT<T>::VEC;
     constexpr bool POOLB = KIND == FPD_EWM_MAXPOOL_BWD;
@@ -369,6 +380,7 @@
     in_t xf = reinterpret_cast<const T*>(POOLB ? m.pool.x : m.full.x);
     in_t gf = reinterpret_cast<const T*>(m.full.dy);
     in_t af = reinterpret_cast<const T*>(APF ? m.full.add : m.pool.add);
+    in_t af2 = reinterpret_cast<const T*>(m.full.add2);
     in_t xh = reinterpret_cast<const T*>(m.half.x);
     in_t gh = reinterpret_cast<const T*>(m.half.dy);
     in_t ah = reinterpret_cast<const T*>(POOLB ? m.half.add : m.pool.add);
@@ -385,9 +397,12 @@
         if (POOLB || APF) { rx0 = ldraw<T>(xf + i00); rx1 = ldraw<T>(xf + i01); rx2 = ldraw<T>(xf + i10); rx3 = ldraw<T>(xf + i11); }
         if (APF) { rg0 = ldraw<T>(gf + i00); rg1 = ldraw<T>(gf + i01); rg2 = ldraw<T>(gf + i10); rg3 = ldraw<T>(gf + i11); }
         if (ADDF) { ra0 = ldraw<T>(af + i00); ra1 = ldraw<T>(af + i01); ra2 = ldraw<T>(af + i10); ra3 = ldraw<T>(af + i11); }
+        uint4 rb0 = z, rb1 = z, rb2 = z, rb3 = z;
+        if (ADD2) { rb0 = ldraw<T>(af2 + i00); rb1 = ldraw<T>(af2 + i01); rb2 = ldraw<T>(af2 + i10); rb3 = ldraw<T>(af2 + i11); }
         if (POOLB) { rxh = ldraw<T>(xh + ih); rgh = ldraw<T>(gh + ih); }
         if (ADDH) rah = ldraw<T>(ah + ih);
         float a0[VEC], a1[VEC], a2[VEC], a3[VEC];
+        if (ADD2) { ra0 = add_raw<T>(ra0, rb0); ra1 = add_raw<T>(ra1, rb1); ra2 = add_raw<T>(ra2, rb2); ra3 = add_raw<T>(ra3, rb3); }
         if (APF) {
             apply_vec<T, ADDF>(rg0, rx0, ra0, s_f, cv, a0);
             apply_vec<T, ADDF>(rg1, rx1, ra1, s_f, cv, a1);
@@ -428,16 +443,90 @@
 
 int g_ew_merge_blocks = 2048;
 
-template <typename T, int KIND, bool FULL, bool ADDF, bool ADDH>
+template <typename T, int KIND, bool FULL, bool ADDF, bool ADDH, bool ADD2 = false>
 int launch_ew_merge(const fpd_ew_merge_t& m, hipStream_t st) {
     const int grid = std::min(ew_rule<T, FPD_EW_SUMPOOL>(m.pool), g_ew_merge_blocks);
-    FPD_LAUNCH((ew_merge_kernel<T, KIND, FULL, ADDF, ADDH>), dim3(grid), dim3(256), 0, st, m);
+    FPD_LAUNCH((ew_merge_kernel<T, KIND, FULL, ADDF, ADDH, ADD2>), dim3(grid), dim3(256), 0, st, m);
     return 0;
 }
 
+template <typename T, bool ADD>
+__global__ __launch_bounds__(256) void ew_apply_bnrelu_bwd_kernel(const fpd_ew_merge_t m) {
+    constexpr int VEC = DT<T>::VEC;
+    __shared__ ApplyTab s_a;
+    __shared__ float s_t0[FPD_MAXC], s_t1[FPD_MAXC], s_t2[FPD_MAXC], s_t3[FPD_MAXC];
+    __shared__ long long s_sum[4 * FPD_MAXC];
+    const fpd_ew_t& a = m.pool;
+    const int tid = threadIdx.x;
+    const int C = a.C, npix = a.N * a.H * a.W;
+    const double cnt = (double)a.N * a.H * a.W;
+    for (int c = tid; c < C; c += 256) {
+        float sc, sh, mu, is;
+        bn_coef(a.bn, c, C, cnt, sc, sh, mu, is);
+        s_t0[c] = sc; s_t1[c] = sh; s_t2[c] = mu; s_t3[c] = is;
+    }
+    apply_tab_fill(m.full, s_a, tid, 256, blockIdx.x == 0);
+    for (int c = tid; c < 4 * C; c += 256) s_sum[c] = 0;
+    __syncthreads();
+    const int VP = C / VEC, PB = 256 / VP;
+    const int cv = (tid % VP) * VEC, pl = tid / VP;
+    const bool active = pl < PB;
+    double acc1[VEC], acc2[VEC];
+#pragma unroll
+    for (int j = 0; j < VEC; ++j) { acc1[j] = 0.0; acc2[j] = 0.0; }
+    typedef const T* __restrict__ in_t;
+    in_t x = reinterpret_cast<const T*>(a.x);
+    in_t x2 = reinterpret_cast<const T*>(a.x2);
+    in_t xf = reinterpret_cast<const T*>(m.full.x);
+    in_t gf = reinterpret_cast<const T*>(m.full.dy);
+    in_t af = reinterpret_cast<const T*>(m.full.add);
+    T* __restrict__ const y = reinterpret_cast<T*>(a.y);
+    if (active) {
+        for (int pix = blockIdx.x * PB + pl; pix < npix; pix += gridDim.x * PB) {
+            const size_t i = (size_t)pix * C + cv;
+            const uint4 z = make_uint4(0u, 0u, 0u, 0u);
+            const uint4 rv = ldraw<T>(x + i), rxf = ldraw<T>(xf + i), rgf = ldraw<T>(gf + i), raf = ADD ? ldraw<T>(af + i) : z;
+            float v[VEC], g[VEC], mk[VEC], o[VEC];
+            DT<T>::unpack(rv, v);
+            if (x2 != nullptr) {
+                ldv<T>(x2 + i, mk);
+            } else {
+#pragma unroll
+                for (int j = 0; j < VEC; ++j) mk[j] = a.bn.relu ? fmaf(v[j], s_t0[cv + j], s_t1[cv + j]) : 1.f;
+            }
+            apply_vec<T, ADD>(rgf, rxf, raf, s_a, cv, g);
+#pragma unroll
+            for (int j = 0; j < VEC; ++j) {
+                o[j] = mk[j] > 0.f ? g[j] : 0.f;
+                const double r = (double)DT<T>::rnd(o[j]);
+                acc1[j] += r;
+                acc2[j] += r * (double)((v[j] - s_t2[cv + j]) * s_t3[cv + j]);
+            }
+            if (y != nullptr) stv<T>(y + i, o);
+        }
+#pragma unroll
+        for (int j = 0; j < VEC; ++j) { stat_lds_add(s_sum, C, 0, cv + j, acc1[j]); stat_lds_add(s_sum, C, 1, cv + j, acc2[j]); }
+    }
+    __syncthreads();
+    for (int c = tid; c < C; c += 256) stat_flush_lds(a.bstats, s_sum, C, c);
+}
+
+template <typename T>
+int launch_ew_apply_bnrelu_bwd(const fpd_ew_merge_t& m, hipStream_t st) {
+    const int grid = ew_grid<T, FPD_EW_BNRELU_BWD_R>(m.pool);
+    if (m.full.add) FPD_LAUNCH((ew_apply_bnrelu_bwd_kernel<T, true>), dim3(grid), dim3(256), 0, st, m);
+    else FPD_LAUNCH((ew_apply_bnrelu_bwd_kernel<T, false>), dim3(grid), dim3(256), 0, st, m);
+    return 0;
+}
+
 template <typename T>
 int dispatch_ew_merge(const fpd_ew_merge_t& m, hipStream_t st) {
+    if (m.kind == FPD_EWM_BNRELU_BWD_R) return launch_ew_apply_bnrelu_bwd<T>(m, st);
     const bool pb = m.kind == FPD_EWM_MAXPOOL_BWD;
+    if (m.full.add2) {
+        return m.half.add ? launch_ew_merge<T, FPD_EWM_MAXPOOL_BWD, true, true, true, true>(m, st)
+                          : launch_ew_merge<T, FPD_EWM_MAXPOOL_BWD, true, true, false, true>(m, st);
+    }
     const bool full = !pb || m.has_full;
     const int v = (pb ? 8 : 0) | (full ? 4 : 0) | ((full ? m.full.add : m.pool.add) ? 2 : 0) | ((pb ? m.half.add : m.pool.add) ? 1 : 0);
     switch (v) {
@@ -478,6 +567,7 @@
 
 static int ew_check(const fpd_ew_t& a) {
     const int vec = (a.dtype == FPD_BF16) ? 8 : 4;
+    if (a.add2) return fpd_fail(-3, "elementwise: add2 is formed by fpd_ew_merge() only (fpd_ew_merge_supported())");
     if (a.C % vec != 0 || a.C > FPD_MAXC || a.C / vec > 128)
         return fpd_fail(-3, "elementwise: C=%d must be a multiple of %d and <= %d", a.C, vec, FPD_MAXC);
     return 0;
@@ -496,6 +586,7 @@
     const int vec = (a.dtype == FPD_BF16) ? 8 : 4;
     if (a.C % vec != 0 || a.C > FPD_MAXC || a.C / vec > 128)
         return fpd_fail(-3, "elementwise: C=%d must be a multiple of %d and <= %d", a.C, vec, FPD_MAXC);
+    if (a.add2) return fpd_fail(-3, "elementwise: add2 is formed by fpd_ew_merge() only (fpd_ew_merge_supported())");
     const bool pooled = (a.op == FPD_EW_MAXPOOL_FWD || a.op == FPD_EW_MAXPOOL_BWD || a.op == FPD_EW_SUMPOOL ||
                          a.op == FPD_EW_UPADD_FWD || a.op == FPD_EW_DILATE2);
     if (pooled && ((a.H & 1) || (a.W & 1))) return fpd_fail(-3, "elementwise: 2x2 ops need even H,W (got %dx%d)", a.H, a.W);
@@ -513,6 +604,17 @@
     return prev;
 }
 
+static int fold_rest_default() {
+    const char* e = getenv("FPD_FOLD_REST");
+    return (e && e[0] == '0' && e[1] == 0) ? 0 : 1;
+}
+static int g_fold_rest = fold_rest_default();
+int fpd_fold_rest_option(int value) {
+    const int prev = g_fold_rest;
+    if (value >= 0) g_fold_rest = value ? 1 : 0;
+    return prev;
+}
+
 int fpd_ew_merge_blocks_option(int value) {
     const int prev = g_ew_merge_blocks;
     if (value >= 1) g_ew_merge_blocks = value;
@@ -534,12 +636,31 @@
 const char* fpd_ew_merge_why_not(const fpd_ew_merge_t& m) {
     if (fpd_ew_merge_option(-1) == 0) return "switched off (FPD_EW_MERGE=0 / option ew_merge)";
     const fpd_ew_t& p = m.pool;
-    if (m.kind != FPD_EWM_MAXPOOL_BWD && m.kind != FPD_EWM_SUMPOOL) return "unknown kind";
+    if (m.kind != FPD_EWM_MAXPOOL_BWD && m.kind != FPD_EWM_SUMPOOL && m.kind != FPD_EWM_BNRELU_BWD_R) return "unknown kind";
     if (p.dtype != FPD_BF16 && p.dtype != FPD_F32) return "bad dtype";
     const int vec = (p.dtype == FPD_BF16) ? 8 : 4;
-    if (p.N <= 0 || p.H <= 0 || p.W <= 0 || p.C <= 0 || (p.H & 1) || (p.W & 1)) return "dims must be positive, H and W even";
+    const bool br = m.kind == FPD_EWM_BNRELU_BWD_R;
+    if (p.N <= 0 || p.H <= 0 || p.W <= 0 || p.C <= 0 || (!br && ((p.H & 1) || (p.W & 1)))) return "dims must be positive, H and W even";
     if (p.C % vec != 0 || p.C > FPD_MAXC || p.C / vec > 128) return "C must be a multiple of the 16-byte vector and <= FPD_MAXC";
     if ((int64_t)p.N * p.H * p.W * p.C >= ((int64_t)1 << 31)) return "tensor too large for 32-bit pixel indexing";
+    if ((br || m.full.add2 || m.half.add2 || p.add2) && fpd_fold_rest_option(-1) == 0) return "switched off (FPD_FOLD_REST=0 / option fold_rest)";
+    if (m.half.add2 || p.add2) return "add2 belongs to the full-resolution apply only";
+    if (m.full.add2 && !(m.kind == FPD_EWM_MAXPOOL_BWD && m.has_full && m.full.add)) return "add2 needs FPD_EWM_MAXPOOL_BWD with the full-resolution apply and its add";
+    if (br) {
+        if (p.op != FPD_EW_BNRELU_BWD_R || !p.x || !p.dy || !p.bstats || p.add || p.out_stats) return "pool member: not a complete FPD_EW_BNRELU_BWD_R";
+        if (!p.bn.gamma || !p.bn.beta || !((p.bn.mode == FPD_BN_TRAIN && p.bn.stats) || (p.bn.mode == FPD_BN_EVAL && p.bn.running_mean && p.bn.running_var)))
+            return "pool member: incomplete BatchNorm";
+        if (!ew_apply_ok(m.full, p, 1)) return "full member is not a complete FPD_EW_BN_BWD_APPLY on [N,H,W,C]";
+        if (p.dy != m.full.y) return "the mask-and-sums pass's dy is not the apply's result";
+        if (p.bstats == m.full.bstats) return "the two members share their backward sums";
+        const void* in[5] = {p.x, p.x2, m.full.x, m.full.dy, m.full.add};
+        for (int i = 0; i < 5; ++i) {
+            if (in[i] != nullptr && in[i] == p.y) return "an output is one of the inputs";
+            if (((uintptr_t)in[i] & 15) != 0) return "pointers must be 16-byte aligned";
+        }
+        if (((uintptr_t)p.y & 15) != 0) return "pointers must be 16-byte aligned";
+        return nullptr;
+    }
     const bool pb = m.kind == FPD_EWM_MAXPOOL_BWD;
     if (p.op != (pb ? FPD_EW_MAXPOOL_BWD : FPD_EW_SUMPOOL) || !p.x || !p.y) return "pool member: wrong op or null pointer";
     const void* in[10];
@@ -552,7 +673,7 @@
         if (m.has_full) {
             if (!ew_apply_ok(m.full, p, 1)) return "full-resolution member is not a complete FPD_EW_BN_BWD_APPLY on [N,H,W,C]";
             if (p.add != m.full.y || p.x != m.full.x) return "the pool backward's add / x are not the full-resolution apply's result / input";
-            in[n++] = m.full.dy; in[n++] = m.full.add;
+            in[n++] = m.full.dy; in[n++] = m.full.add; in[n++] = m.full.add2;
         } else {
             in[n++] = p.add;
         }
diff --git a/fast-human-pose-estimation.pytorch_amd/executor.py b/fast-human-pose-estimation.pytorch_amd/executor.py
--- a/fast-human-pose-estimation.pytorch_amd/executor.py
+++ b/fast-human-pose-estimation.pytorch_amd/executor.py
@@ -272,14 +272,90 @@
                 return False
         return True
 
+    def plan_rest(self, ops):
+        if os.environ.get('FPD_FOLD_REST', '1') == '0':
+            return
+        l = R.lib()
+        live = lambda bs: [b for b in bs if b is not None]
+        for j, op in enumerate(ops):
+            if op is None or op.kind != 'ew' or (op.lane or 0) != 0:
+                continue
+            full = op.ewm_full
+            if op.ewm_kind == 'maxpool_bwd' and full is not None and full.add is not None and op.rest_add is None:
+                made = [i for i in range(j) if ops[i] is not None and any(_abuf(t) is _abuf(full.add) for t in ops[i].acts_out())]
+                i = made[-1] if made else None
+                ad = ops[i] if made else None
+                if ad is None or ad.kind != 'ew' or ad.op != 'add' or (ad.lane or 0) != 0 or ad.absorbed() or tuple(ad.dims) != tuple(full.dims):
+                    continue
+                if any(_abuf(ad.y) is _abuf(t) for t in (ad.x, ad.x2)):
+                    continue
+                if any(_readers_of(ops[i:], ad.y, exclude=(ad, full))):
+                    continue
+                moved = live([_abuf(ad.x), _abuf(ad.x2)])
+                if not self._rest_intervals_ok(moved, [], live([_abuf(op.y)]), ops[i + 1:j]):
+                    continue
+                op.rest_add = ad
+                if l.fpd_ew_merge_supported(C.byref(self.ew_merge(op)[1])) == 1:
+                    ad.rest_absorbed = True
+                else:
+                    op.rest_add = None
+            elif op.op == 'bnrelu_bwd_r' and op.ewm_kind is None and op.rest_apply is None and op.add is None:
+                before = [i for i in range(j) if ops[i] is not None and (ops[i].lane or 0) == 0]
+                i = before[-1] if before else None
+                ap = ops[i] if before else None
+                if ap is None or ap.kind != 'ew' or ap.op != 'bn_bwd_apply' or ap.absorbed() or tuple(ap.dims) != tuple(op.dims):
+                    continue
+                if _abuf(ap.y) is not _abuf(op.dy):
+                    continue
+                if any(_readers_of(ops[i:], ap.y, exclude=(ap, op))):
+                    continue
+                r, w = ap.accesses()
+                outs = live([_abuf(op.y), op.bstats, ap.dgamma, ap.dbeta])
+                moved_wr = live([ap.dgamma, ap.dbeta])
+                if any(self._hit(o, b) for o in outs for b in r + [ap.bstats] + live([_abuf(op.x), _abuf(op.x2)])):
+                    continue
+                if not self._rest_intervals_ok(r + [ap.bstats], moved_wr, [], ops[i + 1:j]):
+                    continue
+                op.rest_apply = ap
+                if l.fpd_ew_merge_supported(C.byref(self.ew_merge(op)[1])) == 1:
+                    ap.rest_absorbed = True
+                else:
+                    op.rest_apply = None
+
+    @staticmethod
+    def _hit(p, q):
+        return p.arena == q.arena and p.off < q.off + q.numel and q.off < p.off + p.numel
+
+    @classmethod
+    def _rest_intervals_ok(cls, moved_rd, moved_wr, outs, between):
+        if any(cls._hit(o, b) for o in outs for b in moved_rd):
+            return False
+        for top in between:
+            if top is None:
+                continue
+            acc = top.accesses()
+            if acc is None:
+                return False
+            r, w = acc
+            if any(cls._hit(a, b) for a in w for b in moved_rd + moved_wr) or any(cls._hit(a, b) for a in r for b in moved_wr):
+                return False
+        return True
+
     def ew_merge(self, op):
         s = R.EwMergeT()
+        if op.rest_apply is not None:
+            s.kind, s.has_full = R.EWM_BNRELU_BWD_R, 1
+            s.full = self.ew(op.rest_apply, plain=True)[1]
+            s.pool = self.ew(op, plain=True)[1]
+            return R.OP_EW_MERGE, s
         s.kind = R.EWM_MAXPOOL_BWD if op.ewm_kind == 'maxpool_bwd' else R.EWM_SUMPOOL
         if op.ewm_full is not None:
             s.has_full, s.full = 1, self.ew(op.ewm_full, plain=True)[1]
         if op.ewm_half is not None:
             s.half = self.ew(op.ewm_half, plain=True)[1]
         s.pool = self.ew(op, plain=True)[1]
+        if op.rest_add is not None:
+            s.full.add, s.full.add2 = self.A.ptr(_abuf(op.rest_add.x)), self.A.ptr(_abuf(op.rest_add.x2))
         return R.OP_EW_MERGE, s
 
     def _fill_skip(self, op, s):
@@ -479,7 +555,7 @@
     def ew(self, op, plain=False):
         if op.absorbed(merged=not plain):
             return _nop()
-        if not plain and op.ewm_kind is not None:
+        if not plain and (op.ewm_kind is not None or op.rest_apply is not None):
             return self.ew_merge(op)
         s = R.EwT()
         s.op, s.dtype = _EW[op.op], self.dtype
@@ -697,6 +773,7 @@
             self.low.plan_folds(bwd_ir)
             if not isinstance(g, G.HRNetGraph):
                 self.low.plan_ew_merge(bwd_ir)
+                self.low.plan_rest(bwd_ir)
             lowered = [self.low.op(op) for op in bwd_ir]
             self.low.finish_partials()
             self.bucket_ops = {}
diff --git a/fast-human-pose-estimation.pytorch_amd/graph.py b/fast-human-pose-estimation.pytorch_amd/graph.py
--- a/fast-human-pose-estimation.pytorch_amd/graph.py
+++ b/fast-human-pose-estimation.pytorch_amd/graph.py
@@ -70,7 +70,9 @@
 class Op:
     PAIRS = ('conv2', 'ew2', 'bneck2')
     fold_apply = fold_wgrad = fused_wgrad = skip_conv = act_ew = w8 = w8s = folded = ewm_kind = ewm_full = ewm_half = upadd_op = x2 = None
+    rest_add = rest_apply = None
     fold_active = fold_other_readers = fused_active = skip_active = skip_fused = act_active = stem_fused = ewm_absorbed = upadd_absorbed = False
+    rest_absorbed = False
 
     def __init__(self, kind, **kw):
         self.kind = kind
@@ -83,7 +85,8 @@
         return [self]
 
     def absorbed(self, merged=True):
-        return bool(self.skip_fused or self.upadd_absorbed or self.stem_fused or (self.kind == 'ew' and self.folded) or (merged and self.ewm_absorbed))
+        return bool(self.skip_fused or self.upadd_absorbed or self.stem_fused or (self.kind == 'ew' and self.folded) or
+                    (merged and (self.ewm_absorbed or self.rest_absorbed)))
 
     def accesses(self):
         def b(a):
@@ -148,6 +151,12 @@
                     if m is not None:
                         rd += [b(m.x), b(m.dy), b(m.add)] + bn_bufs(m.bn)
                         wr += [b(m.y), m.bstats, m.dgamma, m.dbeta]
+            if self.rest_add is not None:
+                rd += [b(self.rest_add.x), b(self.rest_add.x2)]
+            if self.rest_apply is not None:
+                m = self.rest_apply
+                rd += [b(m.x), b(m.dy), b(m.add)] + bn_bufs(m.bn)
+                wr += [m.bstats, m.dgamma, m.dbeta]
         else:
             return None
         return [x for x in rd if x is not None], [x for x in wr if x is not None]
diff --git a/fast-human-pose-estimation.pytorch_amd/runtime.py b/fast-human-pose-estimation.pytorch_amd/runtime.py
--- a/fast-human-pose-estimation.pytorch_amd/runtime.py
+++ b/fast-human-pose-estimation.pytorch_amd/runtime.py
@@ -13,7 +13,7 @@
 (OP_CONV, OP_WGRAD, OP_STEM_FWD, OP_STEM_WGRAD, OP_EW, OP_LOSS, OP_ADAM, OP_MEMSET, OP_WPREP, OP_BNUPD,
  OP_WREDUCE, OP_BNECK, OP_BNECK_FOLD, OP_CONV_PAIR, OP_BNECK_PAIR, OP_EW_PAIR, OP_PCK, OP_HEAD, OP_HEAD_FOLD,
  OP_NOP, OP_AFFSUM, OP_NCHW2NHWC, OP_CONV_F8, OP_WQUANT, OP_LOSS_OHKM, OP_SGD, OP_EW_MERGE, OP_LOSS_KL) = range(28)
-EWM_MAXPOOL_BWD, EWM_SUMPOOL = 0, 1
+EWM_MAXPOOL_BWD, EWM_SUMPOOL, EWM_BNRELU_BWD_R = 0, 1, 2
 AFFSUM_MAX = 4
 MAX_STACKS = 8
 MAX_JOINTS = 32
@@ -74,7 +74,7 @@
 class EwT(C.Structure):
     _fields_ = [('op', _i32), ('dtype', _i32), ('N', _i32), ('H', _i32), ('W', _i32), ('C', _i32), ('x', _vp),
                 ('x2', _vp), ('dy', _vp), ('add', _vp), ('y', _vp), ('out_stats', _vp), ('bstats', _vp),
-                ('dgamma', _vp), ('dbeta', _vp), ('bn', BnT)]
+                ('dgamma', _vp), ('dbeta', _vp), ('bn', BnT), ('add2', _vp)]
 
 
 class EwPairT(C.Structure):
diff --git a/include/fpd_amd.h b/include/fpd_amd.h
--- a/include/fpd_amd.h
+++ b/include/fpd_amd.h
@@ -152,9 +152,10 @@
     float* dgamma;
     float* dbeta;
     fpd_bn_t bn;
+    const void* add2;
 } fpd_ew_t;
 
-enum { FPD_EWM_MAXPOOL_BWD = 0, FPD_EWM_SUMPOOL = 1 };
+enum { FPD_EWM_MAXPOOL_BWD = 0, FPD_EWM_SUMPOOL = 1, FPD_EWM_BNRELU_BWD_R = 2 };
 typedef struct {
     int32_t kind;
     int32_t has_full;
```
